# toposware/certificate-stark

Hardware: AMD Instinct MI355X
Metric: proofs/sec, state_transition AIR @ 2^20 steps (complete prove(): trace gen, LDE, Blake3 commitments, constraint evaluation, composition, DEEP, FRI, 96 queries) (higher is better)
Workload: dtype u64 (63-bit prime field, Montgomery) + u32 (Blake3)

## Files before the change

certificate-stark_amd/csrc/capi.hip:

```cpp
#include <hip/hip_runtime.h>
#include <stdio.h>
#include <stdlib.h>
#include <string.h>
#include <deque>
#include <new>
#include <vector>
#include "../../include/cstark.h"
#include "air_tx_host.h"
#include "blake3.h"
#include "ctx.h"
#include "constraints.h"
#include "deep.h"
#include "ext.h"
#include "generator_fold.h"
#include "hostfield.h"
#include "ntt.h"
#include "trace_gen.h"

namespace cs { thread_local char g_err[512] = ""; }
using cs::fail;
using cs::NttPlan;
using cs::CosetTable;
using cs::PeriodicTable;
using cs::g_err;
// ... 119 lines not shown
int lde_impl_inner(cstark_ctx *c, const uint64_t *d_coeffs, uint64_t *d_lde, uint32_t width, uint32_t col0, uint32_t ncols, uint32_t log_n,
                   uint32_t log_blowup, uint64_t domain_offset, uint32_t k0, uint32_t nk);
template <class F>
int lde_timed(cstark_ctx *c, uint64_t units, F &&run) {
    bool timed = c && c->part_timing && c->lde_ev_used + 2 <= LDE_EVENT_CAP;
    const size_t mark = timed ? c->lde_ev_used : 0;
    if (timed && lde_mark(c) != CSTARK_OK) { c->lde_ev_used = mark; timed = false; }
    const int rc = run();
    if (timed) {
        if (rc == CSTARK_OK && lde_mark(c) == CSTARK_OK) c->lde_units += units;
        else c->lde_ev_used = mark;
    }
    return rc;
}
int lde_impl(cstark_ctx *c, const uint64_t *d_coeffs, uint64_t *d_lde, uint32_t width, uint32_t col0, uint32_t ncols, uint32_t log_n, uint32_t log_blowup,
             uint64_t domain_offset, uint32_t k0, uint32_t nk) {
    return lde_timed(c, (uint64_t)ncols * nk << log_n, [&] { return lde_impl_inner(c, d_coeffs, d_lde, width, col0, ncols, log_n, log_blowup, domain_offset, k0, nk); });
}
int lde_impl_inner(cstark_ctx *c, const uint64_t *d_coeffs, uint64_t *d_lde, uint32_t width, uint32_t col0, uint32_t ncols, uint32_t log_n,
                   uint32_t log_blowup, uint64_t domain_offset, uint32_t k0, uint32_t nk) {
    if (!c || !d_coeffs || !d_lde || width == 0 || ncols == 0 || (uint64_t)col0 + ncols > width) return fail(CSTARK_ERR_INVALID_ARG, "cstark_lde_columns: bad argument");
    if (log_n < cs::NTT_MIN_LOG_N || log_n > cs::NTT_MAX_LOG_N || log_blowup > 6) return fail(CSTARK_ERR_UNSUPPORTED, "unsupported domain size");
    if (domain_offset == 0 || domain_offset >= cs::host::P) return fail(CSTARK_ERR_INVALID_ARG, "domain offset must be a nonzero field element");
    if ((uint64_t)k0 + nk > (1ull << log_blowup)) return fail(CSTARK_ERR_INVALID_ARG, "coset range exceeds the blowup factor");
    HIP_TRY(hipSetDevice(c->device));
    const NttPlan *p;
    const CosetTable *t;
    RC_TRY(get_plan(c, log_n, &p));
    RC_TRY(get_coset_table(c, log_n, log_blowup, domain_offset, &t));
    const size_t n = (size_t)1 << log_n;
    RC_TRY(ensure_ws(c, (size_t)width * n * 8));
    cs::NttArgs a{};
    a.in = d_coeffs + (size_t)col0 * n; a.scratch = (uint64_t *)c->ws;
    a.width = ncols; a.log_n = log_n;
    a.w = p->w; a.do_scale = false; a.aux = p->aux_w;
    if (nk > 1 && (size_t)nk * ncols * n * 8 <= LDE_BATCH_WS_BYTES) {
        if (ensure_ws(c, (size_t)nk * ncols * n * 8) == CSTARK_OK) {
            a.scratch = (uint64_t *)c->ws; a.out = d_lde + (size_t)col0 * n; a.batch = nk;
            a.prescale = t->s + (size_t)k0 * n; a.prescale_batch_stride = n;
            a.aux_ps = t->aux ? t->aux + (size_t)k0 * t->aux_words : nullptr; a.aux_ps_batch_stride = t->aux_words;
            a.in_batch_stride = 0; a.scratch_batch_stride = (size_t)ncols * n; a.out_batch_stride = (size_t)width * n;
            HIP_TRY(cs::ntt_columns(a, c->stream));
            return CSTARK_OK;
        }
        (void)hipGetLastError();
        RC_TRY(ensure_ws(c, (size_t)width * n * 8));
        a.scratch = (uint64_t *)c->ws;
    }
    a.batch = 1;
    for (uint32_t k = k0; k < k0 + nk; k++) {
        a.out = d_lde + ((size_t)(k - k0) * width + col0) * n;
        a.prescale = t->s + (size_t)k * n;
        a.aux_ps = t->aux ? t->aux + (size_t)k * t->aux_words : nullptr;
        HIP_TRY(cs::ntt_columns(a, c->stream));
    }
    return CSTARK_OK;
}

int get_step_table(cstark_ctx *c, unsigned log_n, unsigned log_b, uint64_t offset, unsigned log_block, unsigned split, const cs::StepTable **out) {
    for (const cs::StepTable &t : c->steps)
        if (t.log_n == log_n && t.log_b == log_b && t.offset == offset && t.log_block == log_block && t.split == split) { *out = &t; return CSTARK_OK; }
    const NttPlan *p;
    const CosetTable *ct;
    RC_TRY(get_plan(c, log_n, &p));
    RC_TRY(get_coset_table(c, log_n, log_b, offset, &ct));
    const size_t n = (size_t)1 << log_n, b = (size_t)1 << log_b;
    cs::StepTable t{log_n, log_b, offset, log_block, split, nullptr, nullptr};
    DevGuard g;
    HIP_TRY(g.alloc(&t.d, n * 8));
    HIP_TRY(g.alloc(&t.w, b * n * 8));
    cs::NttArgs a{};
    a.in = t.d; a.scratch = t.w; a.width = 1; a.batch = (unsigned)b; a.log_n = log_n;
    a.w = p->w; a.aux = p->aux_w;
    a.prescale = ct->s; a.prescale_batch_stride = n;
    a.aux_ps = ct->aux; a.aux_ps_batch_stride = ct->aux_words;
    a.in_batch_stride = 0; a.scratch_batch_stride = n;
    HIP_TRY(cs::ntt_step_build_tables(t.d, log_block, split, p->winv, a, c->stream));
    c->steps.push_back(t);
    g.release();
    *out = &c->steps.back();
    return CSTARK_OK;
}
int step_impl(cstark_ctx *c, uint64_t *d_evals, uint64_t *d_coeffs, uint64_t *d_lde, uint32_t width, uint32_t col0, uint32_t ncols, uint32_t log_n,
              uint32_t block_len, uint32_t split, uint32_t log_blowup, uint64_t domain_offset, uint32_t k0, uint32_t nk) {
    if (!c || !d_evals || !d_coeffs || !d_lde || width == 0 || ncols == 0 || (uint64_t)col0 + ncols > width)
        return fail(CSTARK_ERR_INVALID_ARG, "cstark_step_columns: bad argument");
    if (log_n < cs::NTT_MIN_LOG_N || log_n > cs::NTT_MAX_LOG_N || log_blowup > 6) return fail(CSTARK_ERR_UNSUPPORTED, "unsupported domain size");
    if (block_len == 0 || (block_len & (block_len - 1)) || block_len > (1u << log_n)) return fail(CSTARK_ERR_INVALID_ARG, "the block length must be a power of two up to the trace length");
    if (split >= block_len) return fail(CSTARK_ERR_INVALID_ARG, "the split row must lie inside the block");
    if (domain_offset == 0 || domain_offset >= cs::host::P) return fail(CSTARK_ERR_INVALID_ARG, "domain offset must be a nonzero field element");
    if ((uint64_t)k0 + nk > (1ull << log_blowup)) return fail(CSTARK_ERR_INVALID_ARG, "coset range exceeds the blowup factor");
    const size_t n = (size_t)1 << log_n;
    const unsigned log_block = (unsigned)__builtin_ctz(block_len);
    if (!cs::ntt_step_shape(log_n, log_block)) {
        RC_TRY(interpolate_impl(c, d_evals + (size_t)col0 * n, d_coeffs + (size_t)col0 * n, ncols, log_n));
        return lde_impl(c, d_coeffs, d_lde, width, col0, ncols, log_n, log_blowup, domain_offset, k0, nk);
    }
    HIP_TRY(hipSetDevice(c->device));
    const NttPlan *p;
    const cs::StepTable *t;
    RC_TRY(get_plan(c, log_n, &p));
    const cs::StepTable *tr = nullptr;
    RC_TRY(get_step_table(c, log_n, log_blowup, domain_offset, log_block, 0, &t));
    if (split) RC_TRY(get_step_table(c, log_n, log_blowup, domain_offset, log_block, split, &tr));
    RC_TRY(ensure_ws(c, ((size_t)ncols << (log_n - log_block)) * (split ? 16 : 8)));
    uint64_t *fac = (uint64_t *)c->ws;
    if (split)
        HIP_TRY(cs::ntt_step2_coefficients(d_evals + (size_t)col0 * n, fac, d_coeffs + (size_t)col0 * n, t->d, tr->d, ncols, log_n, log_block, split, p->winv,
                                           p->n_inv, c->stream));
    else
        HIP_TRY(cs::ntt_step_coefficients(d_evals + (size_t)col0 * n, fac, d_coeffs + (size_t)col0 * n, t->d, ncols, log_n, log_block, p->winv, p->n_inv, c->stream));
    return lde_timed(c, (uint64_t)ncols * nk << log_n, [&] {
        cs::NttArgs a{};
        a.out = d_lde + (size_t)col0 * n; a.width = ncols; a.batch = nk; a.log_n = log_n;
        a.out_batch_stride = (size_t)width * n; a.aux = p->aux_w;
        HIP_TRY(cs::ntt_step_rows(a, t->w + (size_t)k0 * n, tr ? tr->w + (size_t)k0 * n : nullptr, fac, log_block, c->stream));
        return (int)CSTARK_OK;
    });
}

int extend_periodic_columns(cstark_ctx *c, const std::vector<uint64_t> &cols, uint32_t ncols, uint32_t log_cycle, unsigned log_n, unsigned log_b,
                            DevGuard &keep, uint64_t **d_tab) {
    const size_t words = (size_t)ncols << log_cycle, n = (size_t)1 << log_n;
    uint64_t *d_cols = nullptr, *d_poly = nullptr;
    DevGuard tmp;
    HIP_TRY(tmp.alloc(&d_cols, words * 8));
    HIP_TRY(tmp.alloc(&d_poly, words * 8));
    HIP_TRY(keep.alloc(d_tab, (words << log_b) * 8));
    HIP_TRY(hipMemcpyAsync(d_cols, cols.data(), words * 8, hipMemcpyHostToDevice, c->stream));
    RC_TRY(interpolate_impl(c, d_cols, d_poly, ncols, log_cycle));
    RC_TRY(lde_impl(c, d_poly, *d_tab, ncols, 0, ncols, log_cycle, log_b, cs::host::pow(cs::host::lde_offset(), n >> log_cycle), 0, 1u << log_b));
    HIP_TRY(hipStreamSynchronize(c->stream));
    return CSTARK_OK;
}

int get_periodic(cstark_ctx *c, unsigned depth, unsigned log_n, unsigned log_b, const PeriodicTable **out) {
    for (const PeriodicTable &t : c->periodic)
        if (t.depth == depth && t.log_n == log_n && t.log_b == log_b) { *out = &t; return CSTARK_OK; }
    if (log_n < 10) return fail(CSTARK_ERR_INVALID_ARG, "the trace must hold at least one 1024-row transaction");
    std::vector<uint64_t> cols;
    if (!cs::host::tx_periodic_columns(depth, cols)) return fail(CSTARK_ERR_INVALID_ARG, "unsupported Merkle depth");
    static_assert(cs::host::TX_CYCLE == 1 << 10, "the cycle of TransactionAir's periodic columns");
    const size_t n = (size_t)1 << log_n, b = (size_t)1 << log_b;
    PeriodicTable t{depth, log_n, log_b, nullptr, nullptr, nullptr};
    DevGuard keep;
    RC_TRY(extend_periodic_columns(c, cols, cs::host::TX_NUM_PERIODIC, 10, log_n, log_b, keep, &t.tab));
    HIP_TRY(keep.alloc(&t.coset, b * cs::CE_COSET_CONSTS * 8));
    const uint64_t g = cs::host::lde_offset();
    std::vector<uint64_t> cc(b * cs::CE_COSET_CONSTS);
    const uint64_t wbn = cs::host::root_of_unity(log_n + log_b);
    uint64_t shift = g;
    for (size_t k = 0; k < b; k++) {
        uint64_t *o = cc.data() + k * cs::CE_COSET_CONSTS;
        o[0] = shift;
        o[1] = cs::host::inv(cs::host::sub(cs::host::pow(shift, n), cs::host::ONE));
        for (int gi = 0; gi < 5; gi++) o[2 + gi] = cs::host::pow(shift, cs::host::tx_group_adjustment(gi, n, n * b));
        o[7] = cs::host::pow(shift, cs::host::tx_boundary_adjustment(n, n * b));
        o[8] = cs::host::pow(shift, n - 1);
        o[9] = 0;
        shift = cs::host::mul(shift, wbn);
    }
    HIP_TRY(hipMemcpyAsync(t.coset, cc.data(), cc.size() * 8, hipMemcpyHostToDevice, c->stream));
    const NttPlan *plan;
    RC_TRY(get_plan(c, log_n, &plan));
    HIP_TRY(keep.alloc(&t.binv, b * 2 * n * 8));
    HIP_TRY(cs::build_boundary_inverses(t.binv, plan->w, t.coset, cs::host::inv(cs::host::root_of_unity(log_n)), log_n, log_b, c->stream));
    HIP_TRY(hipStreamSynchronize(c->stream));
    keep.release();
    c->periodic.push_back(t);
    *out = &c->periodic.back();
    return CSTARK_OK;
}

int get_small_periodic(cstark_ctx *c, int air, unsigned depth, unsigned log_n, unsigned log_b, const PeriodicTable **out) {
    for (const PeriodicTable &t : c->small_periodic)
        if (t.air == air && t.depth == depth && t.log_n == log_n && t.log_b == log_b) { *out = &t; return CSTARK_OK; }
    PeriodicTable t{depth, log_n, log_b, nullptr, nullptr, nullptr, air};
    std::vector<uint64_t> cols;
    DevGuard keep;
    if (air == CSTARK_AIR_MERKLE_UPDATE) {
        if (!cs::host::merkle_periodic_columns(depth, cols)) return fail(CSTARK_ERR_INVALID_ARG, "unsupported Merkle depth");
        RC_TRY(extend_periodic_columns(c, cols, 33, 9, log_n, log_b, keep, &t.tab));
    } else if (air == CSTARK_AIR_SCHNORR) {
        cs::host::schnorr_mask_columns(cols);
        RC_TRY(extend_periodic_columns(c, cols, 36, 9, log_n, log_b, keep, &t.tab));
    } else if (air == CSTARK_AIR_RESCUE_CHAIN) {
        using namespace cs::host;
        rescue_chain_periodic_columns(cols);
        const size_t n = (size_t)1 << log_n, b = (size_t)1 << log_b;
        for (int cidx = 0; cidx < 29; cidx++) intt_small(cols.data() + (size_t)cidx * 8, 3);
        std::vector<uint64_t> tab(b * 29 * 8);
        const uint64_t wbn = root_of_unity(log_n + log_b), w8 = root_of_unity(3);
        uint64_t shift = lde_offset();
        for (size_t k = 0; k < b; k++) {
// ... 225 lines not shown
    RC_TRY(tx_witness_reserve(c, n, d, sz, off));
    char *base = (char *)c->wit_buf;
    for (int i = 0; i < cs::WIT_NUM_SEGMENTS; i++)
        if (src[i]) HIP_TRY(hipMemcpyAsync(base + off[i], src[i], sz[i], hipMemcpyHostToDevice, c->stream));
    HIP_TRY(hipStreamSynchronize(c->stream));
    tx_witness_bind(c, n, d, off);
    return CSTARK_OK;
}

int cstark_tx_build_trace(cstark_ctx *c, uint64_t *d_trace) {
    if (!c || !d_trace) return fail(CSTARK_ERR_INVALID_ARG, "cstark_tx_build_trace: null argument");
    if (!c->wit_buf || c->wit.n_tx == 0) return fail(CSTARK_ERR_INVALID_ARG, "no witness uploaded");
    HIP_TRY(hipSetDevice(c->device));
    HIP_TRY(cs::launch_trace_gen(c->wit, d_trace, c->stream, c->side, c->ev_fork, c->ev_join));
    return CSTARK_OK;
}

uint64_t cstark_field_generator(void) { return cs::host::generator(); }
uint64_t cstark_field_lde_offset(void) { return cs::host::lde_offset(); }
uint64_t cstark_field_root_of_unity(uint32_t log_n) { return log_n <= 55 ? cs::host::root_of_unity(log_n) : 0; }

int cstark_interpolate_columns(cstark_ctx *c, uint64_t *d_evals, uint64_t *d_coeffs, uint32_t width, uint32_t log_n) {
    return interpolate_impl(c, d_evals, d_coeffs, width, log_n);
}
int cstark_lde_columns(cstark_ctx *c, const uint64_t *d_coeffs, uint64_t *d_lde, uint32_t width, uint32_t log_n, uint32_t log_blowup,
                       uint64_t domain_offset, uint32_t k0, uint32_t nk) {
    return lde_impl(c, d_coeffs, d_lde, width, 0, width, log_n, log_blowup, domain_offset, k0, nk);
}
int cstark_step_columns(cstark_ctx *c, uint64_t *d_evals, uint64_t *d_coeffs, uint64_t *d_lde, uint32_t width, uint32_t col0, uint32_t ncols,
                        uint32_t log_n, uint32_t block_len, uint32_t log_blowup, uint64_t domain_offset, uint32_t k0, uint32_t nk) {
    return step_impl(c, d_evals, d_coeffs, d_lde, width, col0, ncols, log_n, block_len, 0, log_blowup, domain_offset, k0, nk);
}
int cstark_step2_columns(cstark_ctx *c, uint64_t *d_evals, uint64_t *d_coeffs, uint64_t *d_lde, uint32_t width, uint32_t col0, uint32_t ncols,
                         uint32_t log_n, uint32_t block_len, uint32_t split, uint32_t log_blowup, uint64_t domain_offset, uint32_t k0, uint32_t nk) {
    if (split == 0) return fail(CSTARK_ERR_INVALID_ARG, "the split row must lie inside the block");
    return step_impl(c, d_evals, d_coeffs, d_lde, width, col0, ncols, log_n, block_len, split, log_blowup, domain_offset, k0, nk);
}

int cstark_composition_columns(cstark_ctx *c, const uint64_t *d_combined, uint64_t *d_cols, uint32_t log_n, uint32_t log_blowup) {
    if (!c || !d_combined || !d_cols) return fail(CSTARK_ERR_INVALID_ARG, "cstark_composition_columns: null argument");
    if (log_n < cs::NTT_MIN_LOG_N || log_n + log_blowup > cs::NTT_MAX_LOG_N || log_blowup == 0 || log_blowup > 6)
        return fail(CSTARK_ERR_UNSUPPORTED, "composition domain must be 2^7 .. 2^24 points");
    HIP_TRY(hipSetDevice(c->device));
    const size_t N = (size_t)1 << (log_n + log_blowup);
    RC_TRY(ensure_ws(c, 2 * N * 8));
    uint64_t *nat = (uint64_t *)c->ws, *h = nat + N;
    if (log_blowup <= 3) {
        const NttPlan *pn, *pN;
        RC_TRY(get_plan(c, log_n, &pn));
        RC_TRY(get_plan(c, log_n + log_blowup, &pN));
        cs::NttArgs a{};
        a.in = d_combined; a.scratch = h; a.out = nat; a.width = 1u << log_blowup; a.batch = 1; a.log_n = log_n;
        a.w = pn->winv; a.post_scale = pn->n_inv; a.do_scale = true; a.inverse = true; a.aux = pn->aux_winv;
        HIP_TRY(cs::ntt_columns(a, c->stream));
        const uint64_t b_inv = cs::host::inv(cs::host::from_u64(1ull << log_blowup));
        HIP_TRY(cs::coset_combine(nat, h, log_n, log_blowup, pN->winv, b_inv, c->stream));
        HIP_TRY(cs::split_columns(h, d_cols, log_n, log_blowup, cs::host::inv(cs::host::lde_offset()), c->stream));
        return CSTARK_OK;
    }
    HIP_TRY(cs::interleave_cosets(d_combined, nat, log_n, log_blowup, c->stream));
    const NttPlan *p;
    RC_TRY(get_plan(c, log_n + log_blowup, &p));
    cs::NttArgs a{};
    a.in = nat; a.scratch = nat; a.out = h; a.width = 1; a.batch = 1; a.log_n = log_n + log_blowup;
    a.w = p->winv; a.post_scale = p->n_inv; a.do_scale = true; a.inverse = true; a.aux = p->aux_winv;
    HIP_TRY(cs::ntt_columns(a, c->stream));
    HIP_TRY(cs::split_columns(h, d_cols, log_n, log_blowup, cs::host::inv(cs::host::lde_offset()), c->stream));
    return CSTARK_OK;
}

int cstark_evaluate_polys_at(cstark_ctx *c, const uint64_t *d_coeffs, uint32_t width, uint32_t log_n, const uint64_t *points, uint32_t npts,
                             uint64_t *out ) {
    if (!c || !d_coeffs || !points || !out || width == 0 || npts == 0 || npts > 16) return fail(CSTARK_ERR_INVALID_ARG, "cstark_evaluate_polys_at: bad argument");
    if (log_n > 30) return fail(CSTARK_ERR_INVALID_ARG, "bad polynomial size");
    HIP_TRY(hipSetDevice(c->device));
    const size_t need = ((size_t)npts + (size_t)npts * width + cs::poly_eval_scratch_words(width, log_n, npts)) * 8;
    if (need > c->desc_bytes) {
        if (c->desc_buf) { HIP_TRY(hipStreamSynchronize(c->stream)); HIP_TRY(hipFree(c->desc_buf)); c->desc_buf = nullptr; c->desc_bytes = 0; }
        HIP_TRY(hipMalloc(&c->desc_buf, need));
        c->desc_bytes = need;
    }
    uint64_t *d_pts = (uint64_t *)c->desc_buf, *d_out = d_pts + npts, *d_scr = d_out + (size_t)npts * width;
    HIP_TRY(hipMemcpyAsync(d_pts, points, (size_t)npts * 8, hipMemcpyHostToDevice, c->stream));
    HIP_TRY(cs::poly_eval(d_coeffs, width, log_n, d_pts, npts, d_out, d_scr, c->stream));
    HIP_TRY(hipMemcpyAsync(out, d_out, (size_t)npts * width * 8, hipMemcpyDeviceToHost, c->stream));
    HIP_TRY(cs::stream_wait(c->stream));
    return CSTARK_OK;
}

int cstark_deep_composition(cstark_ctx *c, const uint64_t *d_trace_lde, const uint64_t *d_comp_lde, uint32_t width, uint32_t n_comp,
                            uint64_t z, const uint64_t *ood_trace, const uint64_t *ood_comp, const uint64_t *alpha, const uint64_t *beta,
                            const uint64_t *delta, uint64_t deg_a, uint64_t deg_b, uint64_t *d_out, uint32_t log_n, uint32_t log_blowup,
                            uint32_t k0, uint32_t nk) {
    if (!c || !d_trace_lde || !d_comp_lde || !ood_trace || !ood_comp || !alpha || !beta || !delta || !d_out || nk == 0 || width == 0 || n_comp == 0)
        return fail(CSTARK_ERR_INVALID_ARG, "cstark_deep_composition: bad argument");
    if (log_n < cs::NTT_MIN_LOG_N || log_n > cs::NTT_MAX_LOG_N || log_blowup > 6 || (uint64_t)k0 + nk > (1ull << log_blowup)) return fail(CSTARK_ERR_INVALID_ARG, "bad domain parameters");
    HIP_TRY(hipSetDevice(c->device));
    const NttPlan *plan;
    RC_TRY(get_plan(c, log_n, &plan));
    const size_t b = (size_t)1 << log_blowup, nco = 2 * (size_t)width + n_comp, words = 2 * nco + b;
    if (c->deep_words < words) {
        HIP_TRY(hipStreamSynchronize(c->stream));
        if (c->deep_buf) { HIP_TRY(hipFree(c->deep_buf)); c->deep_buf = nullptr; }
        if (c->deep_stage) { HIP_TRY(hipHostFree(c->deep_stage)); c->deep_stage = nullptr; }
        c->deep_words = 0;
        HIP_TRY(hipMalloc((void **)&c->deep_buf, words * 8));
        HIP_TRY(hipHostMalloc((void **)&c->deep_stage, words * 8, hipHostMallocDefault));
        if (!c->deep_ev) HIP_TRY(hipEventCreateWithFlags(&c->deep_ev, hipEventDisableTiming));
        c->deep_words = words;
    } else {
        HIP_TRY(hipEventSynchronize(c->deep_ev));
    }
    uint64_t *blk = c->deep_stage;
    memcpy(blk, alpha, width * 8); memcpy(blk + width, beta, width * 8); memcpy(blk + 2 * width, delta, n_comp * 8);
    memcpy(blk + nco, ood_trace, 2 * (size_t)width * 8); memcpy(blk + nco + 2 * width, ood_comp, n_comp * 8);
    const uint64_t wbn = cs::host::root_of_unity(log_n + log_blowup);
    uint64_t shift = cs::host::lde_offset();
    for (size_t k = 0; k < b; k++) { blk[2 * nco + k] = shift; shift = cs::host::mul(shift, wbn); }
    HIP_TRY(hipMemcpyAsync(c->deep_buf, blk, words * 8, hipMemcpyHostToDevice, c->stream));
    HIP_TRY(hipEventRecord(c->deep_ev, c->stream));
    const uint64_t *d = c->deep_buf;
    cs::DeepParams p{};
    p.trace_lde = d_trace_lde; p.comp_lde = d_comp_lde; p.w = plan->w; p.coef = d; p.ood = d + nco; p.shifts = d + 2 * nco; p.out = d_out;
    p.z = z; p.zw = cs::host::mul(z, cs::host::root_of_unity(log_n)); p.zb = cs::host::pow(z, n_comp);
    p.deg_a = deg_a; p.deg_b = deg_b; p.width = width; p.nb = n_comp; p.log_n = log_n; p.k0 = k0;
    HIP_TRY(cs::deep_composition(p, nk, c->stream));
    return CSTARK_OK;
}

int cstark_interleave_cosets(cstark_ctx *c, const uint64_t *d_coset_major, uint64_t *d_natural, uint32_t log_n, uint32_t log_blowup) {
    if (!c || !d_coset_major || !d_natural || d_coset_major == d_natural) return fail(CSTARK_ERR_INVALID_ARG, "cstark_interleave_cosets: bad argument");
    if (log_n + log_blowup > 30 || log_blowup > 6) return fail(CSTARK_ERR_INVALID_ARG, "bad domain parameters");
    HIP_TRY(hipSetDevice(c->device));
    HIP_TRY(cs::interleave_cosets(d_coset_major, d_natural, log_n, log_blowup, c->stream));
    return CSTARK_OK;
}
int cstark_fri_fold4(cstark_ctx *c, const uint64_t *d_evals, uint64_t *d_out, uint32_t log_n, uint64_t domain_offset, uint64_t alpha) {
    if (!c || !d_evals || !d_out || d_evals == d_out) return fail(CSTARK_ERR_INVALID_ARG, "cstark_fri_fold4: bad argument");
    if (log_n < cs::NTT_MIN_LOG_N || log_n > cs::NTT_MAX_LOG_N) return fail(CSTARK_ERR_UNSUPPORTED, "layer size must be 2^6 .. 2^24");
    if (domain_offset == 0 || domain_offset >= cs::host::P || alpha >= cs::host::P) return fail(CSTARK_ERR_INVALID_ARG, "offset / alpha must be field elements");
    HIP_TRY(hipSetDevice(c->device));
    const NttPlan *p;
    RC_TRY(get_plan(c, log_n, &p));
    HIP_TRY(cs::fri_fold4(d_evals, d_out, log_n, p->winv, cs::host::inv(domain_offset), alpha, cs::host::inv(cs::host::from_u64(4)), c->stream));
    return CSTARK_OK;
}
int cstark_fri_fold(cstark_ctx *c, const uint64_t *d_evals, uint64_t *d_out, uint32_t log_n, uint32_t folding_factor, uint64_t domain_offset, uint64_t alpha) {
    if (!c || !d_evals || !d_out || d_evals == d_out) return fail(CSTARK_ERR_INVALID_ARG, "cstark_fri_fold: bad argument");
    if (folding_factor != 4 && folding_factor != 8 && folding_factor != 16) return fail(CSTARK_ERR_UNSUPPORTED, "FRI folding factor must be 4, 8 or 16");
    if (log_n < cs::NTT_MIN_LOG_N || log_n > cs::NTT_MAX_LOG_N) return fail(CSTARK_ERR_UNSUPPORTED, "layer size must be 2^6 .. 2^24");
    if (domain_offset == 0 || domain_offset >= cs::host::P || alpha >= cs::host::P) return fail(CSTARK_ERR_INVALID_ARG, "offset / alpha must be field elements");
    HIP_TRY(hipSetDevice(c->device));
    const NttPlan *p;
    RC_TRY(get_plan(c, log_n, &p));
    const unsigned log_f = folding_factor == 4 ? 2 : folding_factor == 8 ? 3 : 4;
    HIP_TRY(cs::fri_fold(d_evals, d_out, log_n, log_f, p->winv, cs::host::inv(domain_offset), alpha, cs::host::inv(cs::host::from_u64(folding_factor)), c->stream));
    return CSTARK_OK;
}

int cstark_evaluate_polys_at_ext(cstark_ctx *c, const uint64_t *d_coeffs, uint32_t width, uint32_t log_n, uint32_t m, const uint64_t *z, uint64_t *out) {
    if (!c || !d_coeffs || !z || !out || width == 0 || (m != 2 && m != 3)) return fail(CSTARK_ERR_INVALID_ARG, "cstark_evaluate_polys_at_ext: bad argument");
    if (log_n > 30) return fail(CSTARK_ERR_INVALID_ARG, "bad polynomial size");
    for (uint32_t i = 0; i < m; i++) if (z[i] >= cs::host::P) return fail(CSTARK_ERR_INVALID_ARG, "the point is not an extension element");
    HIP_TRY(hipSetDevice(c->device));
    const size_t need = ((size_t)m * width + cs::poly_eval_ext_scratch_words(width, log_n, m)) * 8;
    if (need > c->desc_bytes) {
        if (c->desc_buf) { HIP_TRY(hipStreamSynchronize(c->stream)); HIP_TRY(hipFree(c->desc_buf)); c->desc_buf = nullptr; c->desc_bytes = 0; }
        HIP_TRY(hipMalloc(&c->desc_buf, need));
        c->desc_bytes = need;
    }
    uint64_t *d_out = (uint64_t *)c->desc_buf, *d_scr = d_out + (size_t)m * width;
    HIP_TRY(cs::poly_eval_ext(d_coeffs, width, log_n, z, m, d_out, d_scr, c->stream));
    HIP_TRY(hipMemcpyAsync(out, d_out, (size_t)m * width * 8, hipMemcpyDeviceToHost, c->stream));
    HIP_TRY(cs::stream_wait(c->stream));
    return CSTARK_OK;
}
}

int fri_coin_fold_dev(cstark_ctx *c, uint32_t *d_seed, const uint8_t *d_root, uint64_t *d_alpha, uint32_t *d_root_out, const uint64_t *d_evals,
                      uint64_t *d_out, uint32_t log_n, uint32_t log_f, uint64_t domain_offset, uint32_t m) {
    if (log_n < cs::NTT_MIN_LOG_N || log_n > cs::NTT_MAX_LOG_N) return fail(CSTARK_ERR_UNSUPPORTED, "layer size must be 2^6 .. 2^24");
    if (m < 1 || m > 3) return fail(CSTARK_ERR_INVALID_ARG, "fri_coin_fold_dev: bad extension degree");
    const NttPlan *p;
    RC_TRY(get_plan(c, log_n, &p));
    const uint64_t offset_inv = cs::host::inv(domain_offset), inv_f = cs::host::inv(cs::host::from_u64(1ull << log_f));
    if (m == 1) {
        HIP_TRY(cs::fri_coin(d_seed, d_root, d_alpha, d_root_out, c->stream));
        HIP_TRY(cs::fri_fold(d_evals, d_out, log_n, log_f, p->winv, offset_inv, 0, inv_f, c->stream, d_alpha));
    } else {
        HIP_TRY(cs::fri_coin_ext(d_seed, d_root, d_alpha, d_root_out, m, c->stream));
        HIP_TRY(cs::fri_fold_ext(d_evals, d_out, log_n, log_f, p->winv, offset_inv, nullptr, m, inv_f, c->stream, d_alpha));
    }
    return CSTARK_OK;
}
int hash_rows_slots(cstark_ctx *c, uint32_t hash_fn, const uint64_t *d_lde, uint8_t *d_leaves, uint32_t width, uint32_t log_n, uint32_t log_blowup, uint32_t log_s) {
    if (!c || !d_lde || !d_leaves || width == 0 || width > 128 || hash_fn > 1 || log_blowup > 6 || log_s > log_blowup || ((uintptr_t)d_leaves & 15) != 0)
        return fail(CSTARK_ERR_INVALID_ARG, "hash_rows_slots: bad argument");
    HIP_TRY(hipSetDevice(c->device));
    if (hash_fn == 1) HIP_TRY(cs::hash_rows_sha3(d_lde, d_leaves, width, log_n, log_blowup, 0, 1u << log_blowup, c->stream, log_s));
    else HIP_TRY(cs::hash_rows(d_lde, d_leaves, width, log_n, log_blowup, 0, 1u << log_blowup, c->stream, log_s));
    return CSTARK_OK;
}
int evaluate_ood_frames(cstark_ctx *c, const uint64_t *d_coeffs, uint32_t width, const uint64_t *d_ccoef, uint32_t n_comp, uint32_t log_n,
                        const uint64_t zpts[2], uint64_t zb, uint64_t *out_trace, uint64_t *out_comp) {
    if (!c || !d_coeffs || !d_ccoef || !out_trace || !out_comp || width == 0 || n_comp == 0) return fail(CSTARK_ERR_INVALID_ARG, "evaluate_ood_frames: bad argument");
    HIP_TRY(hipSetDevice(c->device));
    const size_t n_out = 2 * (size_t)width + n_comp;
    const size_t scr_t = cs::poly_eval_scratch_words(width, log_n, 2), scr_c = cs::poly_eval_scratch_words(n_comp, log_n, 1);
    const size_t need = (4 + n_out + scr_t + scr_c) * 8;
    if (need > c->desc_bytes) {
        if (c->desc_buf) { HIP_TRY(hipStreamSynchronize(c->stream)); HIP_TRY(hipFree(c->desc_buf)); c->desc_buf = nullptr; c->desc_bytes = 0; }
        HIP_TRY(hipMalloc(&c->desc_buf, need));
        c->desc_bytes = need;
    }
    uint64_t *d_pts = (uint64_t *)c->desc_buf, *d_out = d_pts + 4, *d_scr = d_out + n_out;
    const uint64_t pts[3] = {zpts[0], zpts[1], zb};
    HIP_TRY(hipMemcpyAsync(d_pts, pts, sizeof pts, hipMemcpyHostToDevice, c->stream));
    HIP_TRY(cs::poly_eval(d_coeffs, width, log_n, d_pts, 2, d_out, d_scr, c->stream));
    HIP_TRY(cs::poly_eval(d_ccoef, n_comp, log_n, d_pts + 2, 1, d_out + 2 * (size_t)width, d_scr + scr_t, c->stream));
    std::vector<uint64_t> host(n_out);
    HIP_TRY(hipMemcpyAsync(host.data(), d_out, n_out * 8, hipMemcpyDeviceToHost, c->stream));
    HIP_TRY(cs::stream_wait(c->stream));
    memcpy(out_trace, host.data(), 2 * (size_t)width * 8);
    memcpy(out_comp, host.data() + 2 * (size_t)width, (size_t)n_comp * 8);
    return CSTARK_OK;
}

int ood_frames_dev(cstark_ctx *c, const uint64_t *d_coeffs, uint32_t width, const uint64_t *d_ccoef, uint32_t n_comp, uint32_t log_n, const uint64_t *d_pts,
                   uint64_t *d_out) {
    if (!c || !d_coeffs || !d_ccoef || !d_pts || !d_out || width == 0 || n_comp == 0) return fail(CSTARK_ERR_INVALID_ARG, "ood_frames_dev: bad argument");
    HIP_TRY(hipSetDevice(c->device));
    const size_t scr_t = cs::poly_eval_scratch_words(width, log_n, 2), scr_c = cs::poly_eval_scratch_words(n_comp, log_n, 1);
    const size_t need = (scr_t + scr_c) * 8;
    if (need > c->desc_bytes) {
        if (c->desc_buf) { HIP_TRY(hipStreamSynchronize(c->stream)); HIP_TRY(hipFree(c->desc_buf)); c->desc_buf = nullptr; c->desc_bytes = 0; }
        HIP_TRY(hipMalloc(&c->desc_buf, need));
        c->desc_bytes = need;
    }
    uint64_t *d_scr = (uint64_t *)c->desc_buf;
    HIP_TRY(cs::poly_eval(d_coeffs, width, log_n, d_pts, 2, d_out, d_scr, c->stream));
    HIP_TRY(cs::poly_eval(d_ccoef, n_comp, log_n, d_pts + 2, 1, d_out + 2 * (size_t)width, d_scr + scr_t, c->stream));
    return CSTARK_OK;
}
int desc_reserve(cstark_ctx *c, size_t bytes) {
    if (bytes <= c->desc_bytes) return CSTARK_OK;
    if (c->desc_buf) { HIP_TRY(hipStreamSynchronize(c->stream)); HIP_TRY(hipFree(c->desc_buf)); c->desc_buf = nullptr; c->desc_bytes = 0; }
    HIP_TRY(hipMalloc(&c->desc_buf, bytes));
    c->desc_bytes = bytes;
    return CSTARK_OK;
}
static size_t ood_scratch_words(uint32_t width, uint32_t n_comp, uint32_t log_n, uint32_t m, size_t *scr_t, size_t *scr_c) {
    if (m == 1) { *scr_t = cs::poly_eval_scratch_words(width, log_n, 2); *scr_c = cs::poly_eval_scratch_words(n_comp, log_n, 1); return *scr_t + *scr_c; }
    *scr_t = cs::poly_eval_ext_scratch_words(width, log_n, m); *scr_c = cs::poly_eval_ext_scratch_words(m * n_comp, log_n, m);
    return 2 * *scr_t + *scr_c + (size_t)m * m * n_comp;
}
size_t ood_frames_dev_scratch_bytes(uint32_t width, uint32_t n_comp, uint32_t log_n, uint32_t m) {
    size_t scr_t, scr_c;
    return ood_scratch_words(width, n_comp, log_n, m, &scr_t, &scr_c) * 8;
}
int ood_frames_dev_ext(cstark_ctx *c, const uint64_t *d_coeffs, uint32_t width, const uint64_t *d_ccoef, uint32_t n_comp, uint32_t log_n, uint32_t m,
                       const uint64_t *d_pts, uint64_t *d_out) {
    if (!c || !d_coeffs || !d_ccoef || !d_pts || !d_out || width == 0 || n_comp == 0 || (m != 2 && m != 3)) return fail(CSTARK_ERR_INVALID_ARG, "ood_frames_dev_ext: bad argument");
    HIP_TRY(hipSetDevice(c->device));
    size_t scr_t, scr_c;
    RC_TRY(desc_reserve(c, ood_scratch_words(width, n_comp, log_n, m, &scr_t, &scr_c) * 8));
    uint64_t *d_scr = (uint64_t *)c->desc_buf, *d_raw = d_scr + 2 * scr_t + scr_c;
    const size_t mw = (size_t)m * width;
    HIP_TRY(cs::poly_eval_ext(d_coeffs, width, log_n, nullptr, m, d_out, d_scr, c->stream, d_pts));
    HIP_TRY(cs::poly_eval_ext(d_coeffs, width, log_n, nullptr, m, d_out + mw, d_scr + scr_t, c->stream, d_pts + m));
    HIP_TRY(cs::poly_eval_ext(d_ccoef, m * n_comp, log_n, nullptr, m, d_raw, d_scr + 2 * scr_t, c->stream, d_pts + 2 * m));
    HIP_TRY(cs::ood_recombine_ext(d_raw, d_out + 2 * mw, n_comp, m, c->stream));
    return CSTARK_OK;
}
int deep_composition_ext_dev(cstark_ctx *c, const uint64_t *d_trace_lde, const uint64_t *d_comp_lde, uint32_t width, uint32_t n_comp, uint32_t m,
                             const uint64_t *d_coef, const uint64_t *d_ood, uint64_t *d_scal, const uint64_t *d_shifts, uint64_t *d_out, uint32_t log_n,
                             uint32_t log_blowup, uint32_t nk) {
    if (!c || !d_trace_lde || !d_comp_lde || !d_coef || !d_ood || !d_scal || !d_shifts || !d_out || width == 0 || n_comp == 0 || (m != 2 && m != 3))
        return fail(CSTARK_ERR_INVALID_ARG, "deep_composition_ext_dev: bad argument");
    if (log_n < cs::NTT_MIN_LOG_N || log_n > cs::NTT_MAX_LOG_N || log_blowup > 6 || nk == 0 || nk > (1u << log_blowup)) return fail(CSTARK_ERR_INVALID_ARG, "bad domain parameters");
    HIP_TRY(hipSetDevice(c->device));
    const NttPlan *plan;
    RC_TRY(get_plan(c, log_n, &plan));
    HIP_TRY(cs::deep_ext_consts(d_coef, d_ood, d_scal, width, n_comp, m, c->stream));
    cs::DeepExtParams p{};
    p.trace_lde = d_trace_lde; p.comp_lde = d_comp_lde; p.w = plan->w; p.coef = d_coef; p.shifts = d_shifts; p.out = d_out; p.scal = d_scal;
    p.width = width; p.nb = n_comp; p.log_n = log_n; p.log_b = log_blowup; p.m = m;
    p.nk = nk == (1u << log_blowup) ? 0 : nk;
    HIP_TRY(cs::deep_composition_ext(p, c->stream));
    return CSTARK_OK;
}
int deep_composition_ext_cosets(cstark_ctx *c, const uint64_t *d_trace_lde, const uint64_t *d_comp_lde, uint32_t width, uint32_t n_comp, uint32_t m,
                                const uint64_t *z, const uint64_t *ood_trace, const uint64_t *ood_comp, const uint64_t *alpha, const uint64_t *beta,
                                const uint64_t *delta, const uint64_t *deg_a, const uint64_t *deg_b, uint64_t *d_out, uint32_t log_n, uint32_t log_blowup,
                                uint32_t nk) {
    if (!c || !d_trace_lde || !d_comp_lde || !z || !ood_trace || !ood_comp || !alpha || !beta || !delta || !deg_a || !deg_b || !d_out || width == 0 || n_comp == 0 ||
        (m != 2 && m != 3))
        return fail(CSTARK_ERR_INVALID_ARG, "cstark_deep_composition_ext: bad argument");
    if (log_n < cs::NTT_MIN_LOG_N || log_n > cs::NTT_MAX_LOG_N || log_blowup > 6) return fail(CSTARK_ERR_INVALID_ARG, "bad domain parameters");
    using namespace cs::host;
    HIP_TRY(hipSetDevice(c->device));
    const NttPlan *plan;
    RC_TRY(get_plan(c, log_n, &plan));
    const size_t b = (size_t)1 << log_blowup, nco = (size_t)m * (2 * (size_t)width + n_comp);
    std::vector<uint64_t> blk(nco + b);
    memcpy(blk.data(), alpha, (size_t)m * width * 8);
    memcpy(blk.data() + (size_t)m * width, beta, (size_t)m * width * 8);
    memcpy(blk.data() + (size_t)2 * m * width, delta, (size_t)m * n_comp * 8);
    const uint64_t wbn = root_of_unity(log_n + log_blowup);
    uint64_t shift = lde_offset();
    for (size_t k = 0; k < b; k++) { blk[nco + k] = shift; shift = mul(shift, wbn); }
    const size_t bytes = blk.size() * 8;
    if (bytes > c->desc_bytes) {
        if (c->desc_buf) { HIP_TRY(hipStreamSynchronize(c->stream)); HIP_TRY(hipFree(c->desc_buf)); c->desc_buf = nullptr; c->desc_bytes = 0; }
        HIP_TRY(hipMalloc(&c->desc_buf, bytes));
        c->desc_bytes = bytes;
    }
    HIP_TRY(hipMemcpyAsync(c->desc_buf, blk.data(), bytes, hipMemcpyHostToDevice, c->stream));
    HIP_TRY(cs::stream_wait(c->stream));
    cs::DeepExtParams p{};
    p.trace_lde = d_trace_lde; p.comp_lde = d_comp_lde; p.w = plan->w; p.coef = (const uint64_t *)c->desc_buf; p.shifts = p.coef + nco; p.out = d_out;
    const EX zz = ex_load(z, m), zw = ex_scale(zz, root_of_unity(log_n)), zb = ex_pow(zz, n_comp, m), da = ex_load(deg_a, m), db = ex_load(deg_b, m);
    EX k1 = ex_zero(), k2 = ex_zero(), k3 = ex_zero();
    for (uint32_t i = 0; i < width; i++) {
        k1 = ex_add(k1, ex_mul(ex_load(alpha + (size_t)m * i, m), ex_load(ood_trace + (size_t)m * i, m), m));
// ... 21 lines not shown
int cstark_fri_fold4_ext(cstark_ctx *c, const uint64_t *d_evals, uint64_t *d_out, uint32_t log_n, uint64_t domain_offset, uint32_t m, const uint64_t *alpha) {
    if (!c || !d_evals || !d_out || !alpha || d_evals == d_out || (m != 2 && m != 3)) return fail(CSTARK_ERR_INVALID_ARG, "cstark_fri_fold4_ext: bad argument");
    if (log_n < cs::NTT_MIN_LOG_N || log_n > cs::NTT_MAX_LOG_N) return fail(CSTARK_ERR_UNSUPPORTED, "layer size must be 2^6 .. 2^24");
    if (domain_offset == 0 || domain_offset >= cs::host::P) return fail(CSTARK_ERR_INVALID_ARG, "offset must be a nonzero field element");
    for (uint32_t i = 0; i < m; i++) if (alpha[i] >= cs::host::P) return fail(CSTARK_ERR_INVALID_ARG, "alpha is not an extension element");
    HIP_TRY(hipSetDevice(c->device));
    const NttPlan *p;
    RC_TRY(get_plan(c, log_n, &p));
    HIP_TRY(cs::fri_fold4_ext(d_evals, d_out, log_n, p->winv, cs::host::inv(domain_offset), alpha, m, cs::host::inv(cs::host::from_u64(4)), c->stream));
    return CSTARK_OK;
}
int cstark_fri_fold_ext(cstark_ctx *c, const uint64_t *d_evals, uint64_t *d_out, uint32_t log_n, uint32_t folding_factor, uint64_t domain_offset, uint32_t m,
                        const uint64_t *alpha) {
    if (!c || !d_evals || !d_out || !alpha || d_evals == d_out || (m != 2 && m != 3)) return fail(CSTARK_ERR_INVALID_ARG, "cstark_fri_fold_ext: bad argument");
    if (folding_factor != 4 && folding_factor != 8 && folding_factor != 16) return fail(CSTARK_ERR_UNSUPPORTED, "FRI folding factor must be 4, 8 or 16");
    if (log_n < cs::NTT_MIN_LOG_N || log_n > cs::NTT_MAX_LOG_N) return fail(CSTARK_ERR_UNSUPPORTED, "layer size must be 2^6 .. 2^24");
    if (domain_offset == 0 || domain_offset >= cs::host::P) return fail(CSTARK_ERR_INVALID_ARG, "offset must be a nonzero field element");
    for (uint32_t i = 0; i < m; i++) if (alpha[i] >= cs::host::P) return fail(CSTARK_ERR_INVALID_ARG, "alpha is not an extension element");
    HIP_TRY(hipSetDevice(c->device));
    const NttPlan *p;
    RC_TRY(get_plan(c, log_n, &p));
    const unsigned log_f = folding_factor == 4 ? 2 : folding_factor == 8 ? 3 : 4;
    HIP_TRY(cs::fri_fold_ext(d_evals, d_out, log_n, log_f, p->winv, cs::host::inv(domain_offset), alpha, m, cs::host::inv(cs::host::from_u64(folding_factor)), c->stream));
    return CSTARK_OK;
}

int cstark_hash_rows(cstark_ctx *c, const uint64_t *d_lde, uint8_t *d_leaves, uint32_t width, uint32_t log_n, uint32_t log_blowup,
                     uint32_t k0, uint32_t nk) {
    if (!c || !d_lde || !d_leaves) return fail(CSTARK_ERR_INVALID_ARG, "cstark_hash_rows: null argument");
    if (width == 0 || width > 128) return fail(CSTARK_ERR_UNSUPPORTED, "row width must be 1..128 elements (single Blake3 chunk)");
    if (log_n > 30 || log_blowup > 6 || (uint64_t)k0 + nk > (1ull << log_blowup)) return fail(CSTARK_ERR_INVALID_ARG, "bad domain parameters");
    if (((uintptr_t)d_leaves & 15) != 0) return fail(CSTARK_ERR_INVALID_ARG, "d_leaves must be 16-byte aligned");
    HIP_TRY(hipSetDevice(c->device));
    HIP_TRY(cs::hash_rows(d_lde, d_leaves, width, log_n, log_blowup, k0, nk, c->stream));
    return CSTARK_OK;
}

int cstark_hash_rows_fn(cstark_ctx *c, uint32_t hash_fn, const uint64_t *d_lde, uint8_t *d_leaves, uint32_t width, uint32_t log_n, uint32_t log_blowup,
                        uint32_t k0, uint32_t nk) {
    if (hash_fn == 0) return cstark_hash_rows(c, d_lde, d_leaves, width, log_n, log_blowup, k0, nk);
    if (hash_fn != 1) return fail(CSTARK_ERR_UNSUPPORTED, "hash_fn must be 0 (Blake3_256) or 1 (Sha3_256)");
    if (!c || !d_lde || !d_leaves) return fail(CSTARK_ERR_INVALID_ARG, "cstark_hash_rows_fn: null argument");
    if (width == 0 || width > 128) return fail(CSTARK_ERR_UNSUPPORTED, "row width must be 1..128 elements");
    if (log_n > 30 || log_blowup > 6 || (uint64_t)k0 + nk > (1ull << log_blowup)) return fail(CSTARK_ERR_INVALID_ARG, "bad domain parameters");
    if (((uintptr_t)d_leaves & 15) != 0) return fail(CSTARK_ERR_INVALID_ARG, "d_leaves must be 16-byte aligned");
    HIP_TRY(hipSetDevice(c->device));
    HIP_TRY(cs::hash_rows_sha3(d_lde, d_leaves, width, log_n, log_blowup, k0, nk, c->stream));
    return CSTARK_OK;
}
int cstark_merkle_build_fn(cstark_ctx *c, uint32_t hash_fn, uint8_t *d_nodes, uint32_t log_leaves) {
    if (hash_fn == 0) return cstark_merkle_build(c, d_nodes, log_leaves);
    if (hash_fn != 1) return fail(CSTARK_ERR_UNSUPPORTED, "hash_fn must be 0 (Blake3_256) or 1 (Sha3_256)");
    if (!c || !d_nodes) return fail(CSTARK_ERR_INVALID_ARG, "cstark_merkle_build_fn: null argument");
    if (log_leaves == 0 || log_leaves > 30) return fail(CSTARK_ERR_INVALID_ARG, "tree must have 2 .. 2^30 leaves");
    if (((uintptr_t)d_nodes & 15) != 0) return fail(CSTARK_ERR_INVALID_ARG, "d_nodes must be 16-byte aligned");
    HIP_TRY(hipSetDevice(c->device));
    HIP_TRY(cs::merkle_build_sha3(d_nodes, log_leaves, c->stream));
    return CSTARK_OK;
}

int cstark_merkle_build(cstark_ctx *c, uint8_t *d_nodes, uint32_t log_leaves) {
    if (!c || !d_nodes) return fail(CSTARK_ERR_INVALID_ARG, "cstark_merkle_build: null argument");
    if (log_leaves == 0 || log_leaves > 30) return fail(CSTARK_ERR_INVALID_ARG, "tree must have 2 .. 2^30 leaves");
    if (((uintptr_t)d_nodes & 15) != 0) return fail(CSTARK_ERR_INVALID_ARG, "d_nodes must be 16-byte aligned");
    HIP_TRY(hipSetDevice(c->device));
    HIP_TRY(cs::merkle_build(d_nodes, log_leaves, c->stream));
    return CSTARK_OK;
}

int cstark_tx_evaluate_transitions(cstark_ctx *c, const uint64_t *d_lde, uint64_t *d_out, uint32_t merkle_depth, uint32_t log_n,
                                   uint32_t log_blowup, uint32_t k0, uint32_t nk) {
    cs::CeParams p;
    RC_TRY(ce_params(c, d_lde, d_out, merkle_depth, log_n, log_blowup, k0, nk, &p));
    HIP_TRY(cs::launch_eval_transitions(p, nk, c->stream));
    return CSTARK_OK;
}

}
int lde_column_range(cstark_ctx *c, const uint64_t *d_coeffs, uint64_t *d_lde, uint32_t width, uint32_t col0, uint32_t ncols, uint32_t log_n,
                     uint32_t log_blowup, uint64_t domain_offset, uint32_t k0, uint32_t nk) {
    return lde_impl(c, d_coeffs, d_lde, width, col0, ncols, log_n, log_blowup, domain_offset, k0, nk);
}
int step_column_range(cstark_ctx *c, uint64_t *d_evals, uint64_t *d_coeffs, uint64_t *d_lde, uint32_t width, uint32_t col0, uint32_t ncols, uint32_t log_n,
                      uint32_t block_len, uint32_t split, uint32_t log_blowup, uint64_t domain_offset, uint32_t k0, uint32_t nk) {
    return step_impl(c, d_evals, d_coeffs, d_lde, width, col0, ncols, log_n, block_len, split, log_blowup, domain_offset, k0, nk);
}
int tx_build_trace_split(cstark_ctx *c, uint64_t *d_trace) {
    if (!c || !d_trace) return fail(CSTARK_ERR_INVALID_ARG, "tx_build_trace_split: null argument");
    if (!c->wit_buf || c->wit.n_tx == 0) return fail(CSTARK_ERR_INVALID_ARG, "no witness uploaded");
    HIP_TRY(hipSetDevice(c->device));
    HIP_TRY(cs::launch_trace_gen_split(c->wit, d_trace, c->stream, c->side, c->side2, c->ev_fork, c->ev_join, c->ev_mid, c->ev_join2));
    return CSTARK_OK;
}
static constexpr size_t TX_COEF_WORDS = (size_t)cs::CE_MAX_SETS * cs::CE_COEF_WORDS;
static int ensure_coef_buf(cstark_ctx *c) {
    static_assert(sizeof(cstark_tx_coeffs) == cs::CE_COEF_WORDS * 8, "coefficient block layout");
    if (!c->coef_buf) HIP_TRY(hipMalloc((void **)&c->coef_buf, (TX_COEF_WORDS + (size_t)cs::CE_MAX_SETS * cs::CE_RTAB_WORDS) * 8));
    return CSTARK_OK;
}
int tx_coef_device_block(cstark_ctx *c, uint64_t **d_coef) {
    HIP_TRY(hipSetDevice(c->device));
    RC_TRY(ensure_coef_buf(c));
    *d_coef = c->coef_buf;
    return CSTARK_OK;
}
static int upload_coeffs(cstark_ctx *c, const cstark_tx_coeffs *coeffs, uint32_t m, cs::CeParams &p) {
    constexpr size_t COEF_WORDS = TX_COEF_WORDS;
    RC_TRY(ensure_coef_buf(c));
    if (!c->coef_stage) {
        if (!c->coef_ev) HIP_TRY(hipEventCreateWithFlags(&c->coef_ev, hipEventDisableTiming));
        HIP_TRY(hipHostMalloc(&c->coef_stage, (size_t)cs::CE_MAX_SETS * sizeof(cstark_tx_coeffs), hipHostMallocDefault));
    } else {
        HIP_TRY(hipEventSynchronize(c->coef_ev));
    }
    memcpy(c->coef_stage, coeffs, (size_t)m * sizeof(cstark_tx_coeffs));
    HIP_TRY(hipMemcpyAsync(c->coef_buf, c->coef_stage, (size_t)m * sizeof(cstark_tx_coeffs), hipMemcpyHostToDevice, c->stream));
    HIP_TRY(hipEventRecord(c->coef_ev, c->stream));
    p.coef = c->coef_buf;
    p.rtab = c->coef_buf + COEF_WORDS;
    p.m = m;
    return CSTARK_OK;
}

struct SplitMerge { unsigned log_n = 0; cs::CosetMergeDesc desc; cs::CosetMergeTerm hi; };
static const SplitMerge &tx_split_merge(unsigned log_n) {
    static thread_local SplitMerge sm;
    if (sm.log_n == log_n) return sm;
    const uint64_t n = 1ull << log_n, g = cs::host::lde_offset();
    uint64_t adj[3];
    for (int i = 0; i < 3; i++) adj[i] = cs::host::tx_group_adjustment(i, n, 8 * n);
    static const int first[cs::CE_SPLIT_FAMILIES] = {0, cs::CE_SPLIT_FAM0, 7, 9, 11}, count[cs::CE_SPLIT_FAMILIES] = {4, 3, 2, 2, 2};
    sm.desc = cs::CosetMergeDesc{};
    sm.desc.families = cs::CE_SPLIT_FAMILIES;
    sm.desc.tables_per_set = cs::CE_SPLIT_TABLES;
    sm.desc.raw_family = cs::CE_SPLIT_FAMILIES - 1;
    for (int f = 0; f < cs::CE_SPLIT_FAMILIES; f++) {
        sm.desc.terms[f] = count[f];
        for (int t = 0; t < count[f]; t++) sm.desc.term[f][t] = cs::coset_merge_term(first[f] + t, t ? adj[t - 1] : 0, log_n, g);
    }
    sm.hi = cs::coset_merge_term(0, adj[0], log_n, cs::host::mul(g, cs::host::root_of_unity(log_n + 3)), 2);
    sm.log_n = log_n;
    return sm;
}

namespace {

struct SplitStage {
    unsigned log_n;
    size_t n;
    const NttPlan *pn, *p4, *p8;
    const CosetTable *t1;
    hipStream_t stream;
};
int split_stage(cstark_ctx *c, unsigned log_n, SplitStage *s) {
    *s = SplitStage{log_n, (size_t)1 << log_n, nullptr, nullptr, nullptr, nullptr, c->stream};
    RC_TRY(get_plan(c, log_n, &s->pn));
    RC_TRY(get_plan(c, log_n + 2, &s->p4));
    RC_TRY(get_plan(c, log_n + 3, &s->p8));
    return get_coset_table(c, log_n, 3, cs::host::from_u64(1), &s->t1);
}

int inverse_columns(const SplitStage &s, const uint64_t *in, uint64_t *scratch, uint64_t *out, unsigned width, unsigned batch = 1, size_t batch_stride = 0) {
    cs::NttArgs a{};
    a.in = in; a.scratch = scratch; a.out = out; a.width = width; a.batch = batch; a.log_n = s.log_n;
    a.in_batch_stride = batch_stride; a.scratch_batch_stride = batch_stride; a.out_batch_stride = batch_stride;
    a.w = s.pn->winv; a.post_scale = s.pn->n_inv; a.do_scale = true; a.inverse = true; a.aux = s.pn->aux_winv;
    HIP_TRY(cs::ntt_columns(a, s.stream));
    return CSTARK_OK;
// ... 710 lines not shown
```

certificate-stark_amd/csrc/ctx.h:

```cpp
#pragma once
#include <stdlib.h>
#include <hip/hip_runtime.h>
#include <stdio.h>
#include <deque>
#include <vector>
#include "../../include/cstark.h"
#include "constraints.h"
#include "trace_gen.h"
#include "witness_layout.h"

#include <chrono>
namespace cs {
inline hipError_t stream_wait(hipStream_t st) {
    static const bool block = [] { const char *e = getenv("CSTARK_SYNC_BLOCK"); return e && atoi(e) != 0; }();
    static const long spin_us = [] { const char *e = getenv("CSTARK_SPIN_US"); return e ? atol(e) : 200L; }();
    if (block || spin_us <= 0) return hipStreamSynchronize(st);
    const auto t0 = std::chrono::steady_clock::now();
    hipError_t e;
    for (unsigned it = 0; (e = hipStreamQuery(st)) == hipErrorNotReady; it++) {
#if defined(__x86_64__) || defined(__i386__)
        __builtin_ia32_pause();
#endif
        if ((it & 15) == 15 && std::chrono::duration_cast<std::chrono::microseconds>(std::chrono::steady_clock::now() - t0).count() > spin_us)
            return hipStreamSynchronize(st);
    }
    return e;
}
inline hipError_t stream_wait_tail(hipStream_t st, hipEvent_t near_end) {
    static const bool block = [] { const char *e = getenv("CSTARK_SYNC_BLOCK"); return e && atoi(e) != 0; }();
    if (block) return hipStreamSynchronize(st);
    hipError_t e = hipEventSynchronize(near_end);
    if (e != hipSuccess) return e;
    const auto t0 = std::chrono::steady_clock::now();
    for (unsigned it = 0; (e = hipStreamQuery(st)) == hipErrorNotReady; it++) {
#if defined(__x86_64__) || defined(__i386__)
        __builtin_ia32_pause();
#endif
        if ((it & 15) == 15 && std::chrono::duration_cast<std::chrono::microseconds>(std::chrono::steady_clock::now() - t0).count() > 5000)
            return hipStreamSynchronize(st);
    }
    return e;
}
}

namespace cs {

extern thread_local char g_err[512];

inline int fail(int code, const char *fmt, const char *detail = "") {
    snprintf(g_err, sizeof g_err, fmt, detail);
    return code;
}
#define HIP_TRY(expr)                                                                                                              \
    do {                                                                                                                           \
        hipError_t e_ = (expr);                                                                                                    \
        if (e_ != hipSuccess) return cs::fail(e_ == hipErrorOutOfMemory ? CSTARK_ERR_OOM : CSTARK_ERR_HIP, #expr ": %s", hipGetErrorString(e_)); \
    } while (0)
#define RC_TRY(expr)            \
    do {                        \
        int rc_ = (expr);       \
        if (rc_) return rc_;    \
    } while (0)

int grind_search(hipStream_t stream, unsigned long long *d_found, const uint8_t seed[32], uint32_t hash_fn, unsigned bits, uint64_t chunk, uint64_t *nonce_out);

struct NttPlan {
    unsigned log_n;
    uint64_t *w, *winv;
    uint64_t n_inv;
    uint64_t *aux_w = nullptr, *aux_winv = nullptr;
};
struct CosetTable {
    unsigned log_n, log_b;
    uint64_t offset;
    uint64_t *s;
    uint64_t *aux = nullptr;
    size_t aux_words = 0;
};
struct StepTable {
    unsigned log_n, log_b;
    uint64_t offset;
    unsigned log_block;
    unsigned split;
    uint64_t *d;
    uint64_t *w;
};
struct PeriodicTable {
    unsigned depth, log_n, log_b;
    uint64_t *tab;
    uint64_t *coset;
    uint64_t *binv;
    int air = 0;
};
struct AssertInverseTable {
    unsigned log_n, log_b;
// ... 39 lines not shown
    int device = 0;
    hipStream_t stream = nullptr;
    bool owns_stream = false;
    hipStream_t side = nullptr, side2 = nullptr;
    hipEvent_t ev_fork = nullptr, ev_join = nullptr, ev_join2 = nullptr, ev_mid = nullptr;
    void *wit_buf = nullptr;
    size_t wit_bytes = 0;
    cs::TxWitnessDev wit{};
    std::deque<cs::NttPlan> plans;
    std::deque<cs::CosetTable> cosets;
    std::deque<cs::StepTable> steps;
    std::deque<cs::PeriodicTable> periodic;
    uint64_t *coef_buf = nullptr;
    uint64_t *gfold_j = nullptr;
    void *coef_stage = nullptr;
    hipEvent_t coef_ev = nullptr;
    std::deque<cs::AssertInverseTable> assert_inv;
    std::deque<cs::AirCombineStatic> air_static;
    uint64_t *air_coef_buf = nullptr, *air_coef_stage = nullptr;
    size_t air_coef_words = 0;
    hipEvent_t air_coef_ev = nullptr;
    uint64_t *deep_buf = nullptr, *deep_stage = nullptr;
    size_t deep_words = 0;
    hipEvent_t deep_ev = nullptr;
    std::deque<cs::PeriodicTable> small_periodic;
    void *desc_buf = nullptr;
    hipEvent_t part_ev[cs::CE_NUM_PARTS + 1] = {};
    bool part_timing = false, part_valid = false;
    std::vector<hipEvent_t> lde_ev;
    size_t lde_ev_used = 0;
    uint64_t lde_units = 0;
    uint64_t *tail_buf = nullptr;
    std::vector<uint64_t> schnorr_rx;
    std::vector<uint64_t> schnorr_av_stage;
    std::vector<uint64_t> schnorr_pub;
    std::vector<uint8_t> schnorr_s;
    uint8_t schnorr_seed[32] = {}, schnorr_seed_key[12] = {};
    size_t tail_bytes = 0;
    size_t desc_bytes = 0;
    cs::ProveArena *arena = nullptr;
    cs::VerifyArena *verify = nullptr;
    void *ws = nullptr;
    size_t ws_bytes = 0;
    uint64_t *shard_bit37 = nullptr;
    size_t shard_bit37_words = 0;
    void *rb_dev = nullptr, *rb_host = nullptr;
    size_t rb_dev_bytes = 0, rb_host_bytes = 0;
    void *sig_buf = nullptr;
    size_t sig_bytes = 0;
};
int signature_check(cstark_ctx *c, const char *who, uint32_t count, const uint64_t *messages, const uint64_t *sig_rx, const uint8_t *sig_s,
                    uint8_t *verdicts, uint64_t *rx_out);
int tx_witness_reserve(cstark_ctx *c, size_t n, size_t d, size_t *sz, size_t *off);
void tx_witness_bind(cstark_ctx *c, size_t n, size_t d, const size_t *off);
int fri_coin_fold_dev(cstark_ctx *c, uint32_t *d_seed, const uint8_t *d_root, uint64_t *d_alpha, uint32_t *d_root_out, const uint64_t *d_evals,
                      uint64_t *d_out, uint32_t log_n, uint32_t log_f, uint64_t domain_offset, uint32_t m);
int hash_rows_slots(cstark_ctx *c, uint32_t hash_fn, const uint64_t *d_lde, uint8_t *d_leaves, uint32_t width, uint32_t log_n, uint32_t log_blowup, uint32_t log_s);
struct cstark_gather_desc {
    const void *src;
    void *out;
    const uint32_t *d_pos, *d_count;
    uint32_t paths, a, log_n, log_b, log_s, count, lvl0;
};
int gather_jobs_launch(cstark_ctx *c, const cstark_gather_desc *jobs, uint32_t n_jobs);
int plan_tables(cstark_ctx *c, unsigned log_n, const uint64_t **w, const uint64_t **winv);

struct cstark_tx_coeffs;
int tx_evaluate_constraints_sets(cstark_ctx *c, const uint64_t *d_lde, const cstark_tx_coeffs *coeffs, uint32_t m, const uint64_t pub_inputs[4],
                                 uint64_t *const *d_outs, uint32_t merkle_depth, uint32_t log_n, uint32_t log_blowup, uint32_t k0, uint32_t nk,
                                 bool input_is_lde, const uint64_t *d_pub = nullptr);
int tx_coef_device_block(cstark_ctx *c, uint64_t **d_coef);
int air_stage(cstark_ctx *c, const cs::AirStageRequest &rq);
int tx_evaluate_constraints_shard(cstark_ctx *c, const uint64_t *d_lde, const uint64_t *d_coeffs, const cstark_tx_coeffs *coeffs, const uint64_t pub_inputs[4],
                                  uint64_t *d_out, uint32_t merkle_depth, uint32_t log_n, uint32_t k0, uint32_t nk);
int tx_shard_combine(cstark_ctx *c, const uint64_t *d_parts, uint64_t *d_out, uint32_t log_n, uint32_t nk);
constexpr uint32_t TX_LATE_COLS = 37;
constexpr uint32_t TX_ROOT_COLS = 58;
constexpr uint32_t TX_COPY_COLS = 65;
constexpr uint32_t TX_STEP_COLS = 27;
int tx_build_trace_split(cstark_ctx *c, uint64_t *d_trace);
int lde_column_range(cstark_ctx *c, const uint64_t *d_coeffs, uint64_t *d_lde, uint32_t width, uint32_t col0, uint32_t ncols, uint32_t log_n,
                     uint32_t log_blowup, uint64_t domain_offset, uint32_t k0, uint32_t nk);
int step_column_range(cstark_ctx *c, uint64_t *d_evals, uint64_t *d_coeffs, uint64_t *d_lde, uint32_t width, uint32_t col0, uint32_t ncols, uint32_t log_n,
                      uint32_t block_len, uint32_t split, uint32_t log_blowup, uint64_t domain_offset, uint32_t k0, uint32_t nk);
int evaluate_ood_frames(cstark_ctx *c, const uint64_t *d_coeffs, uint32_t width, const uint64_t *d_ccoef, uint32_t n_comp, uint32_t log_n,
                        const uint64_t zpts[2], uint64_t zb, uint64_t *out_trace, uint64_t *out_comp);
int ood_frames_dev(cstark_ctx *c, const uint64_t *d_coeffs, uint32_t width, const uint64_t *d_ccoef, uint32_t n_comp, uint32_t log_n, const uint64_t *d_pts,
                   uint64_t *d_out);
int desc_reserve(cstark_ctx *c, size_t bytes);
size_t ood_frames_dev_scratch_bytes(uint32_t width, uint32_t n_comp, uint32_t log_n, uint32_t m);
int ood_frames_dev_ext(cstark_ctx *c, const uint64_t *d_coeffs, uint32_t width, const uint64_t *d_ccoef, uint32_t n_comp, uint32_t log_n, uint32_t m,
                       const uint64_t *d_pts, uint64_t *d_out);
int deep_composition_ext_dev(cstark_ctx *c, const uint64_t *d_trace_lde, const uint64_t *d_comp_lde, uint32_t width, uint32_t n_comp, uint32_t m,
                             const uint64_t *d_coef, const uint64_t *d_ood, uint64_t *d_scal, const uint64_t *d_shifts, uint64_t *d_out, uint32_t log_n,
                             uint32_t log_blowup, uint32_t nk);
int deep_composition_ext_cosets(cstark_ctx *c, const uint64_t *d_trace_lde, const uint64_t *d_comp_lde, uint32_t width, uint32_t n_comp, uint32_t m,
                                const uint64_t *z, const uint64_t *ood_trace, const uint64_t *ood_comp, const uint64_t *alpha, const uint64_t *beta,
                                const uint64_t *delta, const uint64_t *deg_a, const uint64_t *deg_b, uint64_t *d_out, uint32_t log_n, uint32_t log_blowup,
                                uint32_t nk);
```

certificate-stark_amd/csrc/deep.h:

```cpp
#pragma once
#include <hip/hip_runtime.h>
#include <stddef.h>
#include <stdint.h>

namespace cs {

struct DeepParams {
    const uint64_t *trace_lde, *comp_lde;
    const uint64_t *w, *shifts;
    const uint64_t *coef;
    const uint64_t *ood;
    uint64_t *out;
    uint64_t z, zw, zb, deg_a, deg_b;
    uint32_t width, nb, log_n, k0;
    const uint64_t *scal;
};

size_t poly_eval_scratch_words(unsigned width, unsigned log_n, unsigned npts);
hipError_t poly_eval(const uint64_t *d_coeffs, unsigned width, unsigned log_n, const uint64_t *d_points, unsigned npts, uint64_t *d_out,
                     uint64_t *d_scratch, hipStream_t stream);
hipError_t deep_composition(const DeepParams &p, unsigned nk, hipStream_t stream);
hipError_t fri_fold4(const uint64_t *d_evals, uint64_t *d_out, unsigned log_n, const uint64_t *d_winv, uint64_t offset_inv, uint64_t alpha,
                     uint64_t inv4, hipStream_t stream, const uint64_t *d_alpha = nullptr);
hipError_t fri_fold(const uint64_t *d_evals, uint64_t *d_out, unsigned log_n, unsigned log_f, const uint64_t *d_winv, uint64_t offset_inv, uint64_t alpha,
                    uint64_t inv_f, hipStream_t stream, const uint64_t *d_alpha = nullptr);

}
```

certificate-stark_amd/csrc/deep.hip:

```cpp
#include "deep.h"
#include "fp.cuh"

namespace cs {
namespace {

#ifndef CS_PE_SEG
#define CS_PE_SEG 16384
#endif
constexpr int PE_SEG = CS_PE_SEG, PE_MAXPTS = 2;
template <int NP>
__global__ __launch_bounds__(256) void k_poly_eval_partial(const fp *__restrict__ coeffs, size_t n, const fp *__restrict__ points, fp *__restrict__ partial,
                                                           unsigned width, unsigned seg_len) {
    __shared__ fp part[NP][256];
    const unsigned segs = gridDim.x, seg = blockIdx.x, col = blockIdx.y, t = threadIdx.x;
    const fp *c = coeffs + (size_t)col * n + (size_t)seg * seg_len;
    fp z[NP], z256[NP], acc[NP];
#pragma unroll
    for (int p = 0; p < NP; p++) { z[p] = points[p]; z256[p] = fp_pow(z[p], 256); acc[p] = 0; }
    const unsigned per = (seg_len + 255) / 256;
    for (unsigned k = per; k-- > 0;) {
        const fp v = k * 256 + t < seg_len ? c[(size_t)k * 256 + t] : 0;
#pragma unroll
        for (int p = 0; p < NP; p++) acc[p] = fp_add(fp_mul(acc[p], z256[p]), v);
    }
#pragma unroll
    for (int p = 0; p < NP; p++) part[p][t] = fp_mul(acc[p], fp_pow(z[p], (uint64_t)seg * seg_len + t));
    __syncthreads();
    for (int s = 128; s > 0; s >>= 1) {
        if ((int)t < s) {
#pragma unroll
            for (int p = 0; p < NP; p++) part[p][t] = fp_add(part[p][t], part[p][t + s]);
        }
        __syncthreads();
    }
    if (t < NP) partial[((size_t)t * width + col) * segs + seg] = part[t][0];
}
__global__ void k_poly_eval_sum(const fp *__restrict__ partial, fp *__restrict__ out, unsigned total, unsigned segs) {
    const unsigned i = blockIdx.x * blockDim.x + threadIdx.x;
    if (i >= total) return;
    fp a = 0;
    for (unsigned s = 0; s < segs; s++) a = fp_add(a, partial[(size_t)i * segs + s]);
    out[i] = a;
}

__global__ __launch_bounds__(256) void k_deep(DeepParams p) {
    const size_t n = (size_t)1 << p.log_n;
    const size_t j = blockIdx.x * (size_t)256 + threadIdx.x;
    if (j >= n) return;
    const unsigned kk = blockIdx.y;
    const fp x = fp_mul(p.shifts[p.k0 + kk], p.w[j]);
    const fp pz = p.scal ? p.scal[0] : p.z, pzw = p.scal ? p.scal[1] : p.zw, pzb = p.scal ? p.scal[2] : p.zb;
    const fp d1 = fp_sub(x, pz), d2 = fp_sub(x, pzw), d3 = fp_sub(x, pzb);
    const fp inv = fp_inv(fp_mul(fp_mul(d1, d2), d3));
    const fp i1 = fp_mul(inv, fp_mul(d2, d3)), i2 = fp_mul(inv, fp_mul(d1, d3)), i3 = fp_mul(inv, fp_mul(d1, d2));
    Acc128 s1 = acc_zero(), s2 = acc_zero(), s3 = acc_zero();
    const fp *t = p.trace_lde + (size_t)kk * p.width * n + j;
    for (unsigned c = 0; c < p.width; c++) {
        const fp v = t[(size_t)c * n];
        acc_mad(s1, p.coef[c], fp_sub(v, p.ood[c]));
        acc_mad(s2, p.coef[p.width + c], fp_sub(v, p.ood[p.width + c]));
        if ((c & 3) == 3) { acc_fold(s1); acc_fold(s2); }
    }
    acc_fold(s1); acc_fold(s2);
    const fp *h = p.comp_lde + (size_t)kk * p.nb * n + j;
    for (unsigned i = 0; i < p.nb; i++) {
        acc_mad(s3, p.coef[2 * p.width + i], fp_sub(h[(size_t)i * n], p.ood[2 * p.width + i]));
        if ((i & 3) == 3) acc_fold(s3);
    }
    acc_fold(s3);
    fp acc = fp_add(fp_add(fp_mul(acc_reduce(s1), i1), fp_mul(acc_reduce(s2), i2)), fp_mul(acc_reduce(s3), i3));
    const fp dga = p.scal ? p.scal[3] : p.deg_a, dgb = p.scal ? p.scal[4] : p.deg_b;
    p.out[(size_t)kk * n + j] = fp_mul(acc, fp_add(dga, fp_mul(dgb, x)));
}

__global__ __launch_bounds__(256) void k_fri_fold4(const fp *__restrict__ evals, fp *__restrict__ out, size_t q, const fp *__restrict__ winv,
                                                   fp offset_inv, fp alpha, fp inv4, const fp *__restrict__ alpha_dev) {
    const size_t i = blockIdx.x * (size_t)256 + threadIdx.x;
    if (i >= q) return;
    if (alpha_dev) alpha = *alpha_dev;
    const fp v0 = evals[i], v1 = evals[i + q], v2 = evals[i + 2 * q], v3 = evals[i + 3 * q];
    const fp zi = winv[q];
    const fp a = fp_add(v0, v2), b = fp_sub(v0, v2), c = fp_add(v1, v3), d = fp_mul(fp_sub(v1, v3), zi);
    const fp s0 = fp_add(a, c), s2 = fp_sub(a, c), s1 = fp_add(b, d), s3 = fp_sub(b, d);
    const fp r = fp_mul(alpha, fp_mul(offset_inv, winv[i]));
    const fp r2 = fp_sqr(r), r3 = fp_mul(r2, r);
    fp acc = fp_add(fp_add(s0, fp_mul(r, s1)), fp_add(fp_mul(r2, s2), fp_mul(r3, s3)));
    out[i] = fp_mul(acc, inv4);
}

template <int LOG_F>
__global__ __launch_bounds__(256) void k_fri_fold(const fp *__restrict__ evals, fp *__restrict__ out, size_t q, const fp *__restrict__ winv,
                                                  fp offset_inv, fp alpha, fp inv_f, const fp *__restrict__ alpha_dev) {
    constexpr int F = 1 << LOG_F;
    const size_t i = blockIdx.x * (size_t)256 + threadIdx.x;
    if (i >= q) return;
    if (alpha_dev) alpha = *alpha_dev;
    fp v[F];
#pragma unroll
    for (int t = 0; t < F; t++) v[t] = evals[i + (size_t)t * q];
#pragma unroll
    for (int len = F; len >= 2; len >>= 1) {
        const int half = len >> 1, step = F / len;
#pragma unroll
        for (int base = 0; base < F; base += len) {
#pragma unroll
            for (int t = 0; t < half; t++) {
                const fp a = v[base + t], b = v[base + t + half];
                v[base + t] = fp_add(a, b);
                const fp d = fp_sub(a, b);
                v[base + t + half] = (t == 0) ? d : fp_mul(d, winv[(size_t)(t * step) * q]);
            }
        }
    }
    const fp r = fp_mul(alpha, fp_mul(offset_inv, winv[i]));
    fp acc = 0;
#pragma unroll
    for (int k = F - 1; k >= 0; k--) {
        int br = 0;
#pragma unroll
        for (int bit = 0; bit < LOG_F; bit++) br |= ((k >> bit) & 1) << (LOG_F - 1 - bit);
        acc = fp_add(fp_mul(acc, r), v[br]);
    }
    out[i] = fp_mul(acc, inv_f);
}

}

hipError_t fri_fold4(const uint64_t *d_evals, uint64_t *d_out, unsigned log_n, const uint64_t *d_winv, uint64_t offset_inv, uint64_t alpha,
                     uint64_t inv4, hipStream_t stream, const uint64_t *d_alpha) {
    const size_t q = ((size_t)1 << log_n) / 4;
    hipLaunchKernelGGL(k_fri_fold4, dim3((unsigned)((q + 255) / 256)), dim3(256), 0, stream, d_evals, d_out, q, d_winv, offset_inv, alpha, inv4, d_alpha);
    return hipGetLastError();
}
hipError_t fri_fold(const uint64_t *d_evals, uint64_t *d_out, unsigned log_n, unsigned log_f, const uint64_t *d_winv, uint64_t offset_inv, uint64_t alpha,
                    uint64_t inv_f, hipStream_t stream, const uint64_t *d_alpha) {
    if (log_f == 2) return fri_fold4(d_evals, d_out, log_n, d_winv, offset_inv, alpha, inv_f, stream, d_alpha);
    if ((log_f != 3 && log_f != 4) || log_n < log_f) return hipErrorInvalidValue;
    const size_t q = ((size_t)1 << log_n) >> log_f;
    const dim3 grid((unsigned)((q + 255) / 256));
    if (log_f == 3) hipLaunchKernelGGL(k_fri_fold<3>, grid, dim3(256), 0, stream, d_evals, d_out, q, d_winv, offset_inv, alpha, inv_f, d_alpha);
    else hipLaunchKernelGGL(k_fri_fold<4>, grid, dim3(256), 0, stream, d_evals, d_out, q, d_winv, offset_inv, alpha, inv_f, d_alpha);
    return hipGetLastError();
}

size_t poly_eval_scratch_words(unsigned width, unsigned log_n, unsigned npts) {
    const size_t n = (size_t)1 << log_n, seg = n < (size_t)PE_SEG ? n : (size_t)PE_SEG;
    return (size_t)npts * width * (n / seg);
}
hipError_t poly_eval(const uint64_t *d_coeffs, unsigned width, unsigned log_n, const uint64_t *d_points, unsigned npts, uint64_t *d_out,
                     uint64_t *d_scratch, hipStream_t stream) {
    const size_t n = (size_t)1 << log_n;
    const unsigned seg_len = (unsigned)(n < (size_t)PE_SEG ? n : (size_t)PE_SEG), segs = (unsigned)(n / seg_len);
    for (unsigned p0 = 0; p0 < npts; p0 += PE_MAXPTS) {
        const unsigned np = npts - p0 >= 2 ? 2 : 1;
        fp *part = d_scratch + (size_t)p0 * width * segs;
        if (np == 2) hipLaunchKernelGGL(k_poly_eval_partial<2>, dim3(segs, width), dim3(256), 0, stream, d_coeffs, n, d_points + p0, part, width, seg_len);
        else hipLaunchKernelGGL(k_poly_eval_partial<1>, dim3(segs, width), dim3(256), 0, stream, d_coeffs, n, d_points + p0, part, width, seg_len);
    }
    const unsigned total = npts * width;
    hipLaunchKernelGGL(k_poly_eval_sum, dim3((total + 255) / 256), dim3(256), 0, stream, d_scratch, d_out, total, segs);
    return hipGetLastError();
}
hipError_t deep_composition(const DeepParams &p, unsigned nk, hipStream_t stream) {
    const size_t n = (size_t)1 << p.log_n;
    hipLaunchKernelGGL(k_deep, dim3((unsigned)((n + 255) / 256), nk), dim3(256), 0, stream, p);
    return hipGetLastError();
}

}
```

certificate-stark_amd/csrc/ntt.hip:

```cpp
#include "ntt.h"
#include "fp.cuh"
#include "hostfield.h"
#include "../../include/cstark_conventions.h"
#ifdef CS_NTT_NOMATH
#define fp_mul(a, b) ((a) ^ (b))
#define fp_add(a, b) ((a) + (b))
#define fp_sub(a, b) ((a) - (b))
#define fp_sub_lazy(a, b) ((a) - (b))
#endif
#ifndef CS_NTT_SKIP
#define CS_NTT_SKIP 0
#endif

namespace cs {
namespace {

__device__ __forceinline__ fp mb_load(const fp *row, unsigned lane_off, unsigned fake) { return (CS_NTT_SKIP & 16) ? (fp)fake : row[lane_off]; }
__device__ __forceinline__ void mb_store(fp *row, unsigned lane_off, fp val) {
    if (!(CS_NTT_SKIP & 8) || val == 0x123456789abcdefull) row[lane_off] = val;
}
constexpr bool MB_NO_TWIDDLE_FILL = (CS_NTT_SKIP & 1) != 0, MB_NO_PRESCALE = (CS_NTT_SKIP & 2) != 0, MB_NO_OUTPUT_FACTOR = (CS_NTT_SKIP & 4) != 0;

constexpr int NT = 256;

// ... 1110 lines not shown
    return hipGetLastError();
}

bool ntt_step_shape(unsigned log_n, unsigned log_block) {
    NttThreeStepShape s;
    return log_block < log_n && ntt_three_step_shape(log_n, &s) && log_n - log_block <= s.log_c;
}
namespace {
__global__ __launch_bounds__(256) void k_step_d(fp *__restrict__ d, const fp *__restrict__ winv, size_t n, unsigned log_t) {
    const size_t k = blockIdx.x * (size_t)256 + threadIdx.x;
    if (k >= n) return;
    d[k] = k == 0 ? FP_ONE : (k & (((size_t)1 << log_t) - 1)) == 0 ? 0 : fp_inv(fp_sub(winv[k], FP_ONE));
}
__global__ __launch_bounds__(256) void k_step_dr(fp *__restrict__ d, const fp *__restrict__ winv, size_t n, unsigned split, fp r_mont) {
    const size_t k = blockIdx.x * (size_t)256 + threadIdx.x;
    if (k >= n) return;
    d[k] = k == 0 ? r_mont : fp_mul(fp_sub(winv[(k * split) & (n - 1)], FP_ONE), fp_inv(fp_sub(winv[k], FP_ONE)));
}
__global__ __launch_bounds__(NT) void k_step_factors(const fp *__restrict__ evals, fp *__restrict__ fac, unsigned log_n, unsigned log_t,
                                                     const fp *__restrict__ winv, fp n_inv, fp t_inv) {
    extern __shared__ __attribute__((aligned(16))) fp smem[];
    const unsigned T = 1u << log_t, log_block = log_n - log_t;
    fp *tile = smem, *tw = smem + T;
    const fp *col = evals + ((size_t)blockIdx.x << log_n);
    for (unsigned t = threadIdx.x; t < T; t += NT) tile[t] = col[(size_t)t << log_block];
    for (unsigned e = threadIdx.x; e < T / 2; e += NT) tw[e] = winv[(size_t)e << log_block];
    __syncthreads();
    lds_ntt_dif<1>(tile, log_t, tw);
    for (unsigned j = threadIdx.x; j < T; j += NT) {
        const fp g = tile[bitrev(j, log_t)];
        fac[((size_t)blockIdx.x << log_t) + j] = j == 0 ? fp_mul(g, t_inv) : fp_mul(fp_mul(g, n_inv), fp_sub(winv[(size_t)j << log_block], FP_ONE));
    }
}
__global__ __launch_bounds__(NT) void k_step2_factors(const fp *__restrict__ evals, fp *__restrict__ fac, unsigned log_n, unsigned log_t, unsigned split,
                                                      const fp *__restrict__ winv, fp n_inv, fp t_inv) {
    extern __shared__ __attribute__((aligned(16))) fp smem[];
    const unsigned T = 1u << log_t, log_block = log_n - log_t;
    fp *tile = smem, *tile_d = smem + T, *tw = smem + 2 * T;
    const fp *col = evals + ((size_t)blockIdx.x << log_n);
    for (unsigned t = threadIdx.x; t < T; t += NT) {
        const fp v = col[((size_t)t << log_block) + split];
        tile[t] = v;
        tile_d[t] = fp_sub(col[(size_t)t << log_block], v);
    }
    for (unsigned e = threadIdx.x; e < T / 2; e += NT) tw[e] = winv[(size_t)e << log_block];
    __syncthreads();
    lds_ntt_dif<1>(tile, log_t, tw);
    lds_ntt_dif<1>(tile_d, log_t, tw);
    fp *out = fac + ((size_t)blockIdx.x << (log_t + 1));
    for (unsigned j = threadIdx.x; j < T; j += NT) {
        const fp g = tile[bitrev(j, log_t)];
        out[j] = j == 0 ? fp_mul(g, t_inv) : fp_mul(fp_mul(g, n_inv), fp_sub(winv[(size_t)j << log_block], FP_ONE));
        out[T + j] = fp_mul(tile_d[bitrev(j, log_t)], n_inv);
    }
}
__global__ __launch_bounds__(256) void k_step2_coeffs(const fp *__restrict__ fac, const fp *__restrict__ d, const fp *__restrict__ dr, fp *__restrict__ coeffs,
                                                      unsigned log_n, unsigned log_t) {
    const size_t k = blockIdx.x * (size_t)256 + threadIdx.x, j = k & (((size_t)1 << log_t) - 1);
    const fp *f = fac + ((size_t)blockIdx.y << (log_t + 1));
    coeffs[((size_t)blockIdx.y << log_n) + k] = fp_add(fp_mul(f[j], d[k]), fp_mul(f[((size_t)1 << log_t) + j], dr[k]));
}
__global__ __launch_bounds__(256) void k_step_coeffs(const fp *__restrict__ fac, const fp *__restrict__ d, fp *__restrict__ coeffs, unsigned log_n,
                                                     unsigned log_t) {
    const size_t k = blockIdx.x * (size_t)256 + threadIdx.x;
    coeffs[((size_t)blockIdx.y << log_n) + k] = fp_mul(fac[((size_t)blockIdx.y << log_t) + (k & (((size_t)1 << log_t) - 1))], d[k]);
}
}
hipError_t ntt_step_build_tables(uint64_t *d_d, unsigned log_block, unsigned split, const uint64_t *d_winv, const NttArgs &a, hipStream_t stream) {
    if (!ntt_step_shape(a.log_n, log_block) || a.inverse || a.width != 1 || a.in != d_d || split >= (1u << log_block)) return hipErrorInvalidValue;
    const size_t n = (size_t)1 << a.log_n;
    if (split == 0) hipLaunchKernelGGL(k_step_d, dim3((unsigned)(n / 256)), dim3(256), 0, stream, d_d, d_winv, n, a.log_n - log_block);
    else hipLaunchKernelGGL(k_step_dr, dim3((unsigned)(n / 256)), dim3(256), 0, stream, d_d, d_winv, n, split, host::from_u64(split));
    const StepPass columns_only{nullptr, nullptr, 0};
    hipError_t e = hipErrorInvalidValue;
    three_step_size(a.log_n, [&](auto split) { e = launch_three_step<decltype(split), false>(a, stream, &columns_only); });
    return e;
}
hipError_t ntt_step_coefficients(const uint64_t *d_evals, uint64_t *d_fac, uint64_t *d_coeffs, const uint64_t *d_d, unsigned ncols, unsigned log_n,
                                 unsigned log_block, const uint64_t *d_winv, uint64_t n_inv, hipStream_t stream) {
    if (!ntt_step_shape(log_n, log_block) || ncols == 0 || ncols > 65535) return hipErrorInvalidValue;
    const unsigned log_t = log_n - log_block;
    const uint64_t t_inv = host::inv(host::from_u64((uint64_t)1 << log_t));
    hipLaunchKernelGGL(k_step_factors, dim3(ncols), dim3(NT), (size_t)3 * 8 << (log_t - 1), stream, d_evals, d_fac, log_n, log_t, d_winv, n_inv, t_inv);
    hipLaunchKernelGGL(k_step_coeffs, dim3((unsigned)(((size_t)1 << log_n) / 256), ncols), dim3(256), 0, stream, (const fp *)d_fac, d_d, d_coeffs, log_n,
                       log_t);
    return hipGetLastError();
}
hipError_t ntt_step2_coefficients(const uint64_t *d_evals, uint64_t *d_fac, uint64_t *d_coeffs, const uint64_t *d_d, const uint64_t *d_dr, unsigned ncols,
                                  unsigned log_n, unsigned log_block, unsigned split, const uint64_t *d_winv, uint64_t n_inv, hipStream_t stream) {
    if (!ntt_step_shape(log_n, log_block) || ncols == 0 || ncols > 65535 || split == 0 || split >= (1u << log_block)) return hipErrorInvalidValue;
    const unsigned log_t = log_n - log_block;
    const uint64_t t_inv = host::inv(host::from_u64((uint64_t)1 << log_t));
    hipLaunchKernelGGL(k_step2_factors, dim3(ncols), dim3(NT), (size_t)5 * 8 << (log_t - 1), stream, d_evals, d_fac, log_n, log_t, split, d_winv, n_inv, t_inv);
    hipLaunchKernelGGL(k_step2_coeffs, dim3((unsigned)(((size_t)1 << log_n) / 256), ncols), dim3(256), 0, stream, (const fp *)d_fac, d_d, d_dr, d_coeffs,
                       log_n, log_t);
    return hipGetLastError();
}
hipError_t ntt_step_rows(const NttArgs &a, const uint64_t *d_wtab, const uint64_t *d_wtab_r, const uint64_t *d_fac, unsigned log_block, hipStream_t stream) {
    if (!ntt_step_shape(a.log_n, log_block) || a.inverse || !d_wtab || !d_fac) return hipErrorInvalidValue;
    const StepPass rows{d_wtab, d_fac, a.log_n - log_block, d_wtab_r};
    hipError_t e = hipErrorInvalidValue;
    three_step_size(a.log_n, [&](auto split) { e = launch_three_step<decltype(split), false>(a, stream, &rows); });
    return e;
}

hipError_t ntt_power_table(fp *d_table, size_t n, fp base, hipStream_t stream) {
    const size_t threads = (n + CHUNK - 1) / CHUNK;
    hipLaunchKernelGGL(k_power_table, dim3((unsigned)((threads + 255) / 256)), dim3(256), 0, stream, d_table, n, base);
    return hipGetLastError();
}

hipError_t ntt_columns(const NttArgs &a, hipStream_t stream) {
    if (a.log_n < NTT_MIN_LOG_N || a.log_n > NTT_MAX_LOG_N) return hipErrorInvalidValue;
    hipError_t e = hipSuccess;
    if (three_step_size(a.log_n, [&](auto split) {
            using S = decltype(split);
            e = a.inverse ? launch_three_step<S, true>(a, stream) : launch_three_step<S, false>(a, stream);
        }))
        return e;
    return (a.log_n + 1) / 2 <= 11 ? launch<8>(a, stream) : launch<4>(a, stream);
}

}
```

certificate-stark_amd/csrc/prove.hip:

```cpp
#include <hip/hip_runtime.h>
#include <string.h>
#include <algorithm>
#include <atomic>
#include <new>
#include <chrono>
#include <thread>
#include <vector>
#include "../../include/cstark.h"
#include "ctx.h"
#include "blake3.h"
#include "channel.h"
#include "deep.h"
#include "ext.h"
#include "range_batch.h"
#include "hostblake3.h"
#include "keccak.cuh"
#include "air_tx_host.h"
#include "hostfield.h"
#include "coin.h"
#include "proof_layout.h"
#include "transcript.h"

namespace cs {

enum { PROVE_EVENTS = CSTARK_PROVE_NUM_STAGES + 1 };

struct ProveArena {
    int air = -1;
    unsigned log_n = 0, log_b = 0, log_f = 0;
    uint64_t *trace = nullptr, *coeffs = nullptr, *lde = nullptr, *combined = nullptr, *ccoef = nullptr, *clde = nullptr, *deep = nullptr;
    std::vector<void *> extra;
    std::vector<size_t> extra_bytes;
    uint8_t *tnodes = nullptr, *cnodes = nullptr;
    std::vector<uint64_t *> layer;
    std::vector<uint8_t *> lnodes;
    uint32_t *d_pos = nullptr;
    uint64_t *d_pub = nullptr;
    uint64_t *d_shifts = nullptr;
    uint8_t *d_open = nullptr;
    uint64_t *h_pub = nullptr;
    uint8_t *h_open = nullptr;
    size_t h_open_bytes = 0;
    size_t open_bytes = 0;
    hipEvent_t ev[PROVE_EVENTS] = {};
    bool timed = false;
    uint32_t channel = CSTARK_CHANNEL_HOST;
    std::vector<void *> owned;
    struct ProofRun *run = nullptr;
};
void proof_run_free(struct ProofRun *r);

void prove_arena_free(ProveArena *a) {
    if (!a) return;
    proof_run_free(a->run);
    for (void *p : a->owned) (void)hipFree(p);
    if (a->h_pub) (void)hipHostFree(a->h_pub);
    if (a->h_open) (void)hipHostFree(a->h_open);
    for (hipEvent_t e : a->ev) if (e) (void)hipEventDestroy(e);
    delete a;
}
int grind_nonce(cstark_ctx *c, ProveArena *a, const Coin &coin, unsigned bits, uint64_t *nonce_out);

namespace {

__global__ void k_gather_rows(const uint64_t *__restrict__ lde, uint32_t width, uint32_t log_n, uint32_t log_b, const uint32_t *__restrict__ pos,
                              uint64_t *__restrict__ out) {
    const uint32_t q = blockIdx.x, i = pos[q], k = i & ((1u << log_b) - 1), j = i >> log_b;
    for (uint32_t c = threadIdx.x; c < width; c += blockDim.x) out[(size_t)q * width + c] = lde[(((size_t)k * width + c) << log_n) + j];
}
__global__ void k_gather_rows_window(const uint64_t *__restrict__ lde, uint32_t width, uint32_t log_n, uint32_t log_b, uint32_t k0, uint32_t nk,
                                     const uint32_t *__restrict__ pos, uint64_t *__restrict__ out, const uint64_t *__restrict__ sub, uint32_t log_nk) {
    const uint32_t q = blockIdx.x, i = pos[q], k = i & ((1u << log_b) - 1), j = i >> log_b, stride = width + 4 * log_nk;
    const bool mine = k >= k0 && k < k0 + nk;
    for (uint32_t c = threadIdx.x; c < width; c += blockDim.x)
        out[(size_t)q * stride + c] = mine ? lde[(((size_t)(k - k0) * width + c) << log_n) + j] : 0;
    const size_t leaf = ((size_t)nk << log_n) + ((size_t)j << log_nk) + (k - k0);
    for (uint32_t t = threadIdx.x; t < 4 * log_nk; t += blockDim.x)
        out[(size_t)q * stride + width + t] = mine ? sub[4 * ((leaf >> (t >> 2)) ^ 1) + (t & 3)] : 0;
}
__global__ void k_split_shard_rows(const uint64_t *__restrict__ rows, uint32_t width, uint32_t log_nk, uint32_t log_leaves, uint64_t *__restrict__ out_rows,
                                   uint64_t *__restrict__ out_paths) {
    const uint32_t q = blockIdx.x, stride = width + 4 * log_nk;
    for (uint32_t c = threadIdx.x; c < width; c += blockDim.x) out_rows[(size_t)q * width + c] = rows[(size_t)q * stride + c];
    for (uint32_t t = threadIdx.x; t < 4 * log_nk; t += blockDim.x) out_paths[(size_t)q * log_leaves * 4 + t] = rows[(size_t)q * stride + width + t];
}
__global__ void k_interleave_leaves(const uint4 *__restrict__ in, uint4 *__restrict__ out, size_t n, uint32_t log_b) {
    const size_t t = blockIdx.x * (size_t)blockDim.x + threadIdx.x;
    if (t >= (n << (log_b + 1))) return;
    const size_t i = t >> 1, half = t & 1, k = i & ((1u << log_b) - 1), j = i >> log_b;
    out[t] = in[2 * (k * n + j) + half];
}
__global__ void k_gather_paths(const uint4 *__restrict__ nodes, uint32_t log_leaves, const uint32_t *__restrict__ pos, uint4 *__restrict__ out) {
    const uint32_t q = blockIdx.x;
    for (uint32_t t = threadIdx.x; t < 2 * log_leaves; t += blockDim.x) {
        const uint32_t lvl = t >> 1, half = t & 1;
        const size_t node = ((((size_t)1 << log_leaves) + pos[q]) >> lvl) ^ 1;
// ... 6 lines not shown
__global__ void k_gather_batch(GatherBatch b) {
    const GatherJob g = b.job[blockIdx.y];
    const uint32_t q = blockIdx.x;
    if (q >= (g.dcount ? *g.dcount : g.count)) return;
    if (g.kind == 0) {
        const uint64_t *lde = (const uint64_t *)g.src;
        uint64_t *out = (uint64_t *)g.out;
        const uint32_t width = g.a, i = g.pos[q], k = lde_coset_slot(i & ((1u << g.log_b) - 1), g.log_b, g.log_s), j = i >> g.log_b;
        for (uint32_t c = threadIdx.x; c < width; c += blockDim.x) out[(size_t)q * width + c] = lde[(((size_t)k * width + c) << g.log_n) + j];
    } else {
        const uint4 *nodes = (const uint4 *)g.src;
        uint4 *out = (uint4 *)g.out;
        const uint32_t log_leaves = g.a;
        for (uint32_t t = threadIdx.x + 2 * g.lvl0; t < 2 * log_leaves; t += blockDim.x) {
            const uint32_t lvl = t >> 1, half = t & 1;
            const size_t node = ((((size_t)1 << log_leaves) + g.pos[q]) >> lvl) ^ 1;
            out[((size_t)q * log_leaves + lvl) * 2 + half] = nodes[2 * node + half];
        }
    }
}
struct GatherList {
    GatherBatch b{};
    int n = 0;
    uint32_t max_count = 0;
    void rows(const uint64_t *lde, uint32_t width, uint32_t log_n, uint32_t log_b, const uint32_t *pos, void *out, uint32_t count, uint32_t log_s = 0,
              const uint32_t *dcount = nullptr) {
        b.job[n++] = GatherJob{lde, out, pos, 0u, width, log_n, log_b, count, log_s, dcount, 0u};
        if (count > max_count) max_count = count;
    }
    void paths(const uint8_t *nodes, uint32_t log_leaves, const uint32_t *pos, void *out, uint32_t count, const uint32_t *dcount = nullptr, uint32_t lvl0 = 0) {
        b.job[n++] = GatherJob{nodes, out, pos, 1u, log_leaves, 0u, 0u, count, 0u, dcount, lvl0};
        if (count > max_count) max_count = count;
    }
    hipError_t launch(hipStream_t st) {
        if (n == 0 || max_count == 0) return hipSuccess;
        k_gather_batch<<<dim3(max_count, (unsigned)n), 128, 0, st>>>(b);
        return hipGetLastError();
    }
};
__global__ void k_gather_pub(const uint64_t *__restrict__ trace, size_t n, uint64_t *__restrict__ out, uint32_t reg0) {
    const uint32_t t = threadIdx.x;
    if (t < 14) out[t] = trace[(size_t)(reg0 + (t % 7)) * n + (t < 7 ? 0 : n - 1)];
}

template <class T>
int dev_alloc(ProveArena *a, T **p, size_t bytes) {
    HIP_TRY(hipMalloc((void **)p, bytes));
    a->owned.push_back(*p);
    return CSTARK_OK;
}

template <class T>
int arena_extra(cstark_ctx *c, ProveArena *a, size_t slot, T **p, size_t bytes) {
    if (a->extra.size() <= slot) { a->extra.resize(slot + 1, nullptr); a->extra_bytes.resize(slot + 1, 0); }
    if (a->extra[slot] && a->extra_bytes[slot] < bytes) {
        HIP_TRY(hipStreamSynchronize(c->stream));
        void *old = a->extra[slot];
        a->extra[slot] = nullptr; a->extra_bytes[slot] = 0;
        a->owned.erase(std::find(a->owned.begin(), a->owned.end(), old));
        HIP_TRY(hipFree(old));
    }
    if (!a->extra[slot]) {
        void *q;
        HIP_TRY(hipMalloc(&q, bytes));
        a->owned.push_back(q); a->extra[slot] = q; a->extra_bytes[slot] = bytes;
    }
    *p = (T *)a->extra[slot];
    return CSTARK_OK;
}

unsigned ceil_log2(uint64_t x) { unsigned l = 0; while ((1ull << l) < x) l++; return l; }

struct AirJob {
    int air = 0;
    uint32_t width = 0, log_n = 0, log_ce = 0, n_constraints = 0, n_assertions = 0, item = 0;
    std::vector<uint64_t> pub;
    std::vector<uint8_t> pub_bytes;
    int (*build)(cstark_ctx *, ProveArena *, AirJob &) = nullptr;
    int (*combine)(cstark_ctx *, ProveArena *, AirJob &, const uint64_t *ta, const uint64_t *tb, const uint64_t *ba, const uint64_t *bb, uint64_t *out) = nullptr;
    int (*combine_sets)(cstark_ctx *, ProveArena *, AirJob &, unsigned m, const uint64_t *const *ta, const uint64_t *const *tb, const uint64_t *const *ba,
                        const uint64_t *const *bb, uint64_t *const *outs) = nullptr;
    struct ColumnBatch { uint32_t col0, ncols; hipEvent_t wait[2]; uint32_t block = 0, split = 0; };
    std::vector<ColumnBatch> batches;
    const uint64_t *pub_staging = nullptr;
    bool public_ready = false;
    bool evals_ready = false;
    uint32_t k0 = 0, nk = 8;
    bool sharded = false;
    bool dev_channel = false;
    const uint64_t *d_coefs = nullptr;
    const uint64_t *d_avalues = nullptr;
    uint32_t log_b = 3;
    uint64_t seed[7] = {};
    uint64_t number = 0;
    const uint64_t *bits = nullptr;
};

void drop_run(ProveArena *a) {
    if (a && a->run) { proof_run_free(a->run); a->run = nullptr; }
}

int get_arena(cstark_ctx *c, const AirJob &job, unsigned log_b, unsigned log_f, unsigned n_layers, size_t nq, ProveArena **out) {
    drop_run(c->arena);
    if (c->arena && c->arena->air == job.air && c->arena->log_n == job.log_n && c->arena->log_b == log_b && c->arena->log_f == log_f &&
        c->arena->layer.size() == n_layers + 1 && c->arena->open_bytes >= nq) { *out = c->arena; return CSTARK_OK; }
    if (c->arena) { HIP_TRY(hipStreamSynchronize(c->stream)); prove_arena_free(c->arena); c->arena = nullptr; }
    ProveArena *a = new (std::nothrow) ProveArena();
    if (!a) return fail(CSTARK_ERR_OOM, "host allocation failed");
    c->arena = a;
    a->air = job.air; a->log_n = job.log_n; a->log_b = log_b; a->log_f = log_f;
    const size_t n = (size_t)1 << job.log_n, b = (size_t)1 << log_b, N = n * b, W = job.width, ce = (size_t)1 << job.log_ce, f = (size_t)1 << log_f;
    RC_TRY(dev_alloc(a, &a->trace, W * n * 8));
    RC_TRY(dev_alloc(a, &a->coeffs, W * n * 8));
    RC_TRY(dev_alloc(a, &a->lde, W * N * 8));
    RC_TRY(dev_alloc(a, &a->tnodes, 2 * N * 32));
    RC_TRY(dev_alloc(a, &a->combined, N * 8));
    RC_TRY(dev_alloc(a, &a->ccoef, ce * n * 8));
    RC_TRY(dev_alloc(a, &a->clde, b * ce * n * 8));
    RC_TRY(dev_alloc(a, &a->cnodes, 2 * N * 32));
    RC_TRY(dev_alloc(a, &a->deep, N * 8));
    size_t sz = N;
    for (unsigned l = 0; l <= n_layers; l++) {
        uint64_t *e; uint8_t *t = nullptr;
        RC_TRY(dev_alloc(a, &e, sz * 8));
        if (l < n_layers) RC_TRY(dev_alloc(a, &t, 2 * (sz / f) * 32));
        a->layer.push_back(e); a->lnodes.push_back(t);
        sz /= f;
    }
    RC_TRY(dev_alloc(a, &a->d_pos, 4 * 256 * (n_layers + 2)));
    RC_TRY(dev_alloc(a, &a->d_pub, 16 * 8));
    RC_TRY(dev_alloc(a, &a->d_shifts, b * 8));
    {
        std::vector<uint64_t> sh(b);
        const uint64_t wbn = host::root_of_unity(job.log_n + log_b);
        uint64_t v = host::lde_offset();
        for (size_t k = 0; k < b; k++) { sh[k] = v; v = host::mul(v, wbn); }
        HIP_TRY(hipMemcpy(a->d_shifts, sh.data(), b * 8, hipMemcpyHostToDevice));
    }
    a->open_bytes = nq;
    const size_t log_N = job.log_n + log_b;
    const size_t per_q = W * 8 + ce * 8 + 2 * log_N * 32 + (size_t)n_layers * (f * 8 + log_N * 32);
    RC_TRY(dev_alloc(a, &a->d_open, per_q * nq + 256));
    for (hipEvent_t &e : a->ev) HIP_TRY(hipEventCreate(&e));
    *out = a;
    return CSTARK_OK;
}

int check_options(const cstark_options *opt, unsigned log_ce, unsigned *log_rem_out, unsigned *log_b_out, unsigned *log_f_out) {
    const uint32_t b = opt->blowup_factor, f = opt->fri_folding_factor;
    if (b != 2 && b != 4 && b != 8 && b != 16) return fail(CSTARK_ERR_UNSUPPORTED, "blowup_factor must be 2, 4, 8 or 16");
    if (b < (1u << log_ce)) return fail(CSTARK_ERR_INVALID_ARG, "blowup_factor below the AIR's constraint-evaluation blowup (TransactionAir / SchnorrAir 8, MerkleAir 4, RangeProofAir 2)");
    if (opt->hash_fn > 1) return fail(CSTARK_ERR_UNSUPPORTED, "hash_fn must be Blake3_256 (0) or Sha3_256 (1)");
    if (opt->field_extension > 2) return fail(CSTARK_ERR_INVALID_ARG, "field_extension must be None (0), Quadratic (1) or Cubic (2)");
    if (f != 4 && f != 8 && f != 16) return fail(CSTARK_ERR_UNSUPPORTED, "fri_folding_factor must be 4, 8 or 16");
    *log_b_out = b == 2 ? 1 : b == 4 ? 2 : b == 8 ? 3 : 4;
    *log_f_out = f == 4 ? 2 : f == 8 ? 3 : 4;
    if (opt->num_queries == 0 || opt->num_queries > 128) return fail(CSTARK_ERR_INVALID_ARG, "num_queries must be 1..128");
    if (opt->grinding_factor > 32) return fail(CSTARK_ERR_INVALID_ARG, "grinding_factor must be at most 32");
    unsigned log_rem = 0;
    while ((1u << log_rem) < opt->fri_max_remainder) log_rem++;
    if ((1u << log_rem) != opt->fri_max_remainder || log_rem < 7 || log_rem > 10) return fail(CSTARK_ERR_INVALID_ARG, "fri_max_remainder must be a power of two in 128..1024");
    *log_rem_out = log_rem;
    return CSTARK_OK;
}

using transcript::channel_seed;
using transcript::SEED_PREFIX;
std::vector<uint8_t> channel_seed(const AirJob &job, const cstark_options &opt, unsigned log_rem) {
    return channel_seed(job.width, job.log_n, opt, job.log_b, log_rem, job.pub.data(), job.pub.size(), job.pub_bytes.data(), job.pub_bytes.size());
}

struct Queries {
    uint64_t nonce = 1;
    uint32_t counts[VMAX_LAYERS] = {};
    std::vector<uint32_t> hpos;
};
int query_stage(cstark_ctx *c, ProveArena *a, Coin &coin, const ProofShape &S, Queries &Q) {
    RC_TRY(grind_nonce(c, a, coin, S.opt[2], &Q.nonce));
    Q.hpos.assign(256 * (S.n_layers + 1), 0);
    transcript::draw_queries(coin, S, Q.nonce, Q.hpos.data(), Q.hpos.data() + 256, 256, Q.counts);
    HIP_TRY(hipMemcpyAsync(a->d_pos, Q.hpos.data(), Q.hpos.size() * 4, hipMemcpyHostToDevice, c->stream));
    return CSTARK_OK;
}

struct OpenBlock { size_t trows, tpaths, crows, cpaths, lrows[VMAX_LAYERS], lpaths[VMAX_LAYERS], bytes; };
OpenBlock open_block(const ProofShape &S, const uint32_t *counts, size_t start = 0, size_t align = 1) {
    OpenBlock O;
    size_t off = start;
    auto take = [&off, align](size_t bytes) { const size_t o = off; off += (bytes + align - 1) / align * align; return o; };
    O.trows = take(trace_row_bytes(S)); O.tpaths = take(path_bytes(S)); O.crows = take(comp_row_bytes(S)); O.cpaths = take(path_bytes(S));
    for (unsigned l = 0; l < S.n_layers; l++) {
        const uint32_t np = counts ? counts[l] : S.nq;
        O.lrows[l] = take(layer_row_bytes(S, np)); O.lpaths[l] = take(layer_path_bytes(S, l, np));
    }
    O.bytes = off;
    return O;
}
int host_open_block(ProveArena *a, size_t bytes) {
    if (a->h_open_bytes < bytes) {
        if (a->h_open) { HIP_TRY(hipHostFree(a->h_open)); a->h_open = nullptr; a->h_open_bytes = 0; }
        HIP_TRY(hipHostMalloc((void **)&a->h_open, bytes, hipHostMallocDefault));
        a->h_open_bytes = bytes;
    }
    return CSTARK_OK;
}
struct OpenSrc {
    const uint64_t *clde; uint64_t *const *layer; unsigned log_s;
    const uint32_t *counts, *dcount;
    const uint64_t *shard_rows; uint32_t shard_lvl0;
};
int open_stage(cstark_ctx *c, ProveArena *a, const ProofShape &S, const OpenSrc &src, uint8_t *d_block, const OpenBlock &O) {
    hipStream_t st = c->stream;
    const uint32_t nq = S.nq, W = S.width;
    GatherList gl;
    uint32_t trace_lvl0 = 0;
    if (src.shard_rows) {
        trace_lvl0 = src.shard_lvl0;
        k_split_shard_rows<<<nq, 128, 0, st>>>(src.shard_rows, W, trace_lvl0, S.log_N, (uint64_t *)(d_block + O.trows), (uint64_t *)(d_block + O.tpaths));
        HIP_TRY(hipGetLastError());
    } else gl.rows(a->lde, W, S.log_n, S.log_b, a->d_pos, d_block + O.trows, nq, src.log_s);
    gl.paths(a->tnodes, S.log_N, a->d_pos, d_block + O.tpaths, nq, nullptr, trace_lvl0);
    gl.rows(src.clde, S.ce * S.m, S.log_n, S.log_b, a->d_pos, d_block + O.crows, nq);
    gl.paths(a->cnodes, S.log_N, a->d_pos, d_block + O.cpaths, nq);
    for (unsigned l = 0; l < S.n_layers; l++) {
        const uint32_t np = src.counts ? src.counts[l] : nq, lr = layer_log_rows(S, l), *pos = a->d_pos + 256 * (l + 1), *dc = src.dcount ? src.dcount + l : nullptr;
        gl.rows(src.layer[l], S.f * S.m, lr, 0, pos, d_block + O.lrows[l], np, 0, dc);
        gl.paths(a->lnodes[l], lr, pos, d_block + O.lpaths[l], np, dc);
    }
    HIP_TRY(gl.launch(st));
    RC_TRY(host_open_block(a, O.bytes));
    HIP_TRY(hipMemcpyAsync(a->h_open, d_block, O.bytes, hipMemcpyDeviceToHost, st));
    return CSTARK_OK;
}

int lde_trace(cstark_ctx *c, ProveArena *a, const AirJob &job, uint32_t col0, uint32_t ncols) {
    const uint32_t W = job.width, log_n = job.log_n, log_b = job.log_b;
    if (job.sharded || log_b <= job.log_ce) return lde_column_range(c, a->coeffs, a->lde, W, col0, ncols, log_n, log_b, host::lde_offset(), job.k0, job.nk);
    const size_t n = (size_t)1 << log_n, ce = (size_t)1 << job.log_ce;
    const uint64_t wbn = host::root_of_unity(log_n + log_b);
    uint64_t offset = host::lde_offset();
    for (uint32_t r = 0; r < (1u << (log_b - job.log_ce)); r++) {
        RC_TRY(lde_column_range(c, a->coeffs, a->lde + (size_t)r * ce * W * n, W, col0, ncols, log_n, job.log_ce, offset, 0, (uint32_t)ce));
        offset = host::mul(offset, wbn);
    }
    return CSTARK_OK;
}
int commit_columns(cstark_ctx *c, ProveArena *a, AirJob &job, hipStream_t st, int &evi) {
    const uint32_t W = job.width, log_n = job.log_n;
    const size_t n = (size_t)1 << log_n;
    if (job.batches.empty()) {
        RC_TRY(cstark_interpolate_columns(c, a->trace, a->coeffs, W, log_n));
        HIP_TRY(hipEventRecord(a->ev[evi++], st));
        RC_TRY(lde_trace(c, a, job, 0, W));
        HIP_TRY(hipEventRecord(a->ev[evi++], st));
        return CSTARK_OK;
    }
    for (size_t i = 0; i < job.batches.size(); i++) {
        const AirJob::ColumnBatch &cb = job.batches[i];
        for (hipEvent_t e : cb.wait)
            if (e) HIP_TRY(hipStreamWaitEvent(st, e, 0));
        const bool step = cb.block != 0 && !job.sharded && job.log_b <= job.log_ce;
        if (!step) RC_TRY(cstark_interpolate_columns(c, a->trace + (size_t)cb.col0 * n, a->coeffs + (size_t)cb.col0 * n, cb.ncols, log_n));
        if (i + 1 == job.batches.size()) HIP_TRY(hipEventRecord(a->ev[evi++], st));
        if (step) RC_TRY(step_column_range(c, a->trace, a->coeffs, a->lde, W, cb.col0, cb.ncols, log_n, cb.block, cb.split, job.log_b, host::lde_offset(), job.k0, job.nk));
        else RC_TRY(lde_trace(c, a, job, cb.col0, cb.ncols));
    }
    HIP_TRY(hipEventRecord(a->ev[evi++], st));
    return CSTARK_OK;
}

}

int grind_nonce(cstark_ctx *c, ProveArena *a, const Coin &coin, unsigned bits, uint64_t *nonce_out) {
    static const bool dev_env = [] { const char *e = getenv("CSTARK_GRIND_DEVICE"); return !e || atoi(e) != 0; }();
    if (bits == 0 || !dev_env || bits < 12) {
        *nonce_out = transcript::host_nonce(coin, bits);
        return CSTARK_OK;
    }
    unsigned long long *d_found;
    RC_TRY(arena_extra(c, a, 42, &d_found, 64));
    return grind_search(c->stream, d_found, coin.seed, coin.hash_fn, bits, (uint64_t)1 << 22, nonce_out);
}
int grind_search(hipStream_t stream, unsigned long long *d_found, const uint8_t seed[32], uint32_t hash_fn, unsigned bits, uint64_t chunk, uint64_t *nonce_out) {
    if (chunk == 0) return fail(CSTARK_ERR_INVALID_ARG, "proof of work: empty chunk");
    if (hash_fn == 1) {
        HIP_TRY(hipMemcpyAsync(d_found + 1, seed, 32, hipMemcpyHostToDevice, stream));
        HIP_TRY(hipMemsetAsync(d_found, 0xFF, 8, stream));
    }
    for (uint64_t base = 1;; base += chunk) {
        if (hash_fn == 1) HIP_TRY(cs::grind_batch_chunk_sha3((const uint64_t *)(d_found + 1), 1, base, chunk, bits, d_found, stream));
        else HIP_TRY(cs::grind_chunk(seed, base, chunk, bits, d_found, stream));
        unsigned long long found = 0;
        HIP_TRY(hipMemcpyAsync(&found, d_found, 8, hipMemcpyDeviceToHost, stream));
        HIP_TRY(cs::stream_wait(stream));
        if (found != ~0ull) { *nonce_out = found; return CSTARK_OK; }
        if (base > ((uint64_t)1 << 44)) return fail(CSTARK_ERR_HIP, "proof of work: no nonce found");
    }
}

struct ProofRun {
    cstark_options opt{};
    AirJob job;
    unsigned log_rem = 0, n_layers = 0, log_b = 3, log_f = 2, m = 1;
    ProofShape shape{};
    Coin coin;
    uint8_t trace_root[32] = {}, cons_root[32] = {}, rem_commit[32] = {};
    std::vector<uint64_t> ta[3], tb[3], ba[3], bb[3], ood_trace, ood_comp, remainder;
    std::vector<uint8_t> layer_roots;
    uint64_t *comb[3] = {}, *cco[3] = {};
    uint64_t *ccoefs = nullptr;
    uint64_t *clde = nullptr, *deep = nullptr;
    std::vector<uint64_t *> layer;
    uint8_t *d_open = nullptr;
    Queries q;
    int evi = 0, phase = 0;
    bool sharded() const { return job.sharded; }
    unsigned log_s() const { return job.sharded ? 0 : log_b - job.log_ce; }
};
void proof_run_free(ProofRun *r) { delete r; }

namespace {

int run_buffers(cstark_ctx *c, ProveArena *a, ProofRun &R) {
    const unsigned m = R.m, n_layers = R.n_layers, log_N = R.job.log_n + R.log_b;
    if (m == 1) {
        R.comb[0] = a->combined; R.cco[0] = R.ccoefs = a->ccoef; R.clde = a->clde; R.deep = a->deep; R.layer = a->layer; R.d_open = a->d_open;
        return CSTARK_OK;
    }
    const size_t b = (size_t)1 << R.log_b, N = b << R.job.log_n, W = R.job.width, CN = (size_t)1 << (R.job.log_ce + R.job.log_n), nq = R.opt.num_queries;
    const uint32_t fold = 1u << R.log_f;
    uint64_t *combined_x, *ccoef_x;
    RC_TRY(arena_extra(c, a, 16, &combined_x, 2 * CN * 8));
    RC_TRY(arena_extra(c, a, 17, &ccoef_x, 2 * CN * 8));
    RC_TRY(arena_extra(c, a, 18, &R.ccoefs, 3 * CN * 8));
    RC_TRY(arena_extra(c, a, 19, &R.clde, 3 * b * CN * 8));
    RC_TRY(arena_extra(c, a, 20, &R.deep, 3 * N * 8));
    RC_TRY(arena_extra(c, a, 21, &R.d_open, nq * (W * 8 + 192 + 2 * log_N * 32 + (size_t)n_layers * (fold * 24 + log_N * 32)) + 256));
    R.layer.resize(n_layers + 1);
    size_t sz = N;
    for (unsigned l = 0; l <= n_layers; l++) { RC_TRY(arena_extra(c, a, 22 + l, &R.layer[l], 3 * sz * 8)); sz >>= R.log_f; }
    for (unsigned q = 0; q < 3; q++) { R.comb[q] = q ? combined_x + (q - 1) * CN : a->combined; R.cco[q] = q ? ccoef_x + (q - 1) * CN : a->ccoef; }
    return CSTARK_OK;
}

int run_setup(cstark_ctx *c, const cstark_options *opt, const AirJob &job, ProofRun &R, ProveArena **a) {
    RC_TRY(check_options(opt, job.log_ce, &R.log_rem, &R.log_b, &R.log_f));
    const unsigned log_N = job.log_n + R.log_b;
// ... 221 lines not shown
    const bool dev_coin = dev_coin_env && hf == 0 && m == 1 && n_layers > 0;
    uint32_t *d_fri = nullptr, *d_roots = nullptr;
    R.layer_roots.assign(32 * (size_t)n_layers, 0);
    if (dev_coin) {
        RC_TRY(arena_extra(c, a, 41, &d_fri, (size_t)(8 + 10 * 32) * 4));
        HIP_TRY(hipMemcpyAsync(d_fri, coin.seed, 32, hipMemcpyHostToDevice, st));
        d_roots = d_fri + 8 + 2 * 32;
    }
    RC_TRY(fri_commit(c, a, R, d_fri, d_roots, R.layer[n_layers]));
    R.remainder.assign((size_t)m << (log_N - n_layers * R.log_f), 0);
    if (dev_coin) HIP_TRY(hipMemcpyAsync(R.layer_roots.data(), d_roots, 32 * (size_t)n_layers, hipMemcpyDeviceToHost, st));
    HIP_TRY(hipMemcpyAsync(R.remainder.data(), R.layer[n_layers], R.remainder.size() * 8, hipMemcpyDeviceToHost, st));
    HIP_TRY(cs::stream_wait(st));
    if (dev_coin)
        for (unsigned l = 0; l < n_layers; l++) transcript::fri_layer(coin, &R.layer_roots[32 * l], m, nullptr);
    transcript::commit_remainder(coin, R.remainder.data(), R.remainder.size(), R.rem_commit);
    STAGE();

    RC_TRY(query_stage(c, a, coin, R.shape, R.q));
    R.phase = 3;
    return CSTARK_OK;
}

int phase_open(cstark_ctx *c, ProveArena *a, ProofRun &R, const uint64_t *d_trace_rows, uint8_t *proof, size_t capacity, size_t *proof_len) {
    const ProofShape &S = R.shape;
    const OpenBlock O = open_block(S, R.q.counts);
    RC_TRY(open_stage(c, a, S, {R.clde, R.layer.data(), R.log_s(), R.q.counts, nullptr, d_trace_rows, ceil_log2(R.job.nk)}, R.d_open, O));
    STAGE();
    HIP_TRY(cs::stream_wait(c->stream));
    a->timed = true; a->channel = CSTARK_CHANNEL_HOST;

    ProofParts p{};
    p.trace_root = R.trace_root; p.cons_root = R.cons_root; p.layer_roots = R.layer_roots.data(); p.rem_commit = R.rem_commit;
    p.ood_trace = R.ood_trace.data(); p.ood_comp = R.ood_comp.data(); p.nonce = R.q.nonce; p.remainder = R.remainder.data();
    return finish_proof(S, p, a->h_open, O, R.q.counts, proof, capacity, proof_len);
}

int prove_core(cstark_ctx *c, const cstark_options *opt, AirJob &job, uint8_t *proof, size_t capacity, size_t *proof_len) {
    ProofRun R;
    ProveArena *a;
    RC_TRY(run_setup(c, opt, job, R, &a));
    RC_TRY(phase_commit(c, a, R, nullptr));
    RC_TRY(phase_evaluate(c, a, R, nullptr, a->combined));
    RC_TRY(phase_compose(c, a, R));
    return phase_open(c, a, R, nullptr, proof, capacity, proof_len);
}
int prove_core_dev(cstark_ctx *c, const cstark_options *opt, AirJob &job0, uint8_t *proof, size_t capacity, size_t *proof_len) {
    const auto hp0 = std::chrono::steady_clock::now();
    ProofRun R;
    ProveArena *a;
    job0.dev_channel = true;
    RC_TRY(run_setup(c, opt, job0, R, &a));
    AirJob &job = R.job;
    const unsigned m = R.m, log_n = job.log_n, log_b = R.log_b, log_N = log_n + log_b, n_layers = R.n_layers;
    const size_t n = (size_t)1 << log_n, W = job.width, ce = (size_t)1 << job.log_ce, nq = opt->num_queries;
    const size_t rem_len = (size_t)m << (log_N - n_layers * R.log_f), n_ood = m * (2 * W + ce);
    hipStream_t st = c->stream;
    size_t off = 0;
    auto take = [&off](size_t bytes) { const size_t o = off; off += (bytes + 255) & ~(size_t)255; return o; };
    const size_t o_troot = take(32), o_croot = take(32), o_rem = take(32), o_cnt = take(4 * 64), o_ood = take(n_ood * 8), o_lroots = take(32 * (size_t)n_layers),
                 o_remainder = take(rem_len * 8);
    const ProofShape &S = R.shape;
    const OpenBlock O = open_block(S, nullptr, off, 256);
    off = O.bytes;
    uint8_t *d_res;
    uint32_t *d_fri;
    uint64_t *d_chan;
    uint64_t *sums, *dcoef;
    RC_TRY(arena_extra(c, a, 44, &d_res, off));
    RC_TRY(arena_extra(c, a, 43, &d_chan, 12 * m * 8 + n_ood * 8));
    if (m == 1) {
        RC_TRY(arena_extra(c, a, 41, &d_fri, (size_t)(8 + 10 * 32) * 4));
        RC_TRY(arena_extra(c, a, 40, &dcoef, n * 8));
        sums = R.deep;
    } else {
        RC_TRY(arena_extra(c, a, 47, &d_fri, (size_t)(8 + 2 * 3 * 32) * 4));
        RC_TRY(arena_extra(c, a, 48, &sums, 3 * n * 8));
        RC_TRY(arena_extra(c, a, 49, &dcoef, 3 * n * 8));
    }
    uint64_t *d_pts = d_chan, *d_scal = d_chan + 4 * m, *d_deepc = d_chan + 12 * m, *d_ood = (uint64_t *)(d_res + o_ood);
    uint32_t *d_cnt = (uint32_t *)(d_res + o_cnt);
    RC_TRY(host_open_block(a, off));
    RC_TRY(desc_reserve(c, ood_frames_dev_scratch_bytes((uint32_t)W, (uint32_t)ce, log_n, m)));
    uint64_t *d_coef_block;
    const bool is_tx = job.air == CSTARK_AIR_STATE_TRANSITION;
    const size_t coef_stride = is_tx ? (size_t)CE_COEF_WORDS : 230 + 2 * (size_t)job.n_assertions;
    if (is_tx) RC_TRY(tx_coef_device_block(c, &d_coef_block));
    else RC_TRY(arena_extra(c, a, 46, &d_coef_block, m * coef_stride * 8));
    const uint64_t *pw, *pwinv;
    RC_TRY(plan_tables(c, log_n, &pw, &pwinv));

    RC_TRY(commit_trace_leaves(c, a, R));
    RC_TRY(cstark_merkle_build_fn(c, R.opt.hash_fn, a->tnodes, log_N));
    STAGE();
    {
        ChanStep s{};
        s.seed = d_fri; s.m = m;
        const std::vector<uint8_t> prefix = channel_seed(job.width, log_n, *opt, log_b, R.log_rem);
        if (job.air == CSTARK_AIR_SCHNORR) {
            uint8_t key[12] = {};
            memcpy(key, prefix.data(), 2); memcpy(key + 2, prefix.data() + 10, 7); key[11] = 1;
            if (memcmp(key, c->schnorr_seed_key, sizeof key) != 0) {
                const std::vector<uint8_t> seed = channel_seed(job, *opt, R.log_rem);
                hostb3::hash(seed.data(), seed.size(), c->schnorr_seed);
                memcpy(c->schnorr_seed_key, key, sizeof key);
            }
            HIP_TRY(hipMemcpyAsync(d_fri, c->schnorr_seed, 32, hipMemcpyHostToDevice, st));
        } else {
            s.init = 1; s.pub = a->d_pub; s.npub = job.air == CSTARK_AIR_RANGE ? 1 : 14;
        }
        memcpy(s.prefix, prefix.data(), SEED_PREFIX); s.prefix_len = SEED_PREFIX;
        s.absorb[0].kind = CHAN_DIGEST; s.absorb[0].ptr = a->tnodes + 32; s.absorb[0].copy_out = d_res + o_troot;
        s.draw = CHAN_DRAW_COEFFS; s.a = job.n_constraints; s.b = job.n_assertions; s.stride = CSTARK_TX_NUM_CONSTRAINTS;
        s.set_stride = (uint32_t)coef_stride;
        s.count = (uint32_t)transcript::coefficient_draws(job.n_constraints, job.n_assertions); s.out = d_coef_block;
        HIP_TRY(channel_step(s, st));
    }
    if (is_tx) {
        RC_TRY(tx_evaluate_constraints_sets(c, a->lde, nullptr, m, nullptr, R.comb, job.item, log_n, 3, 0, 8, true, a->d_pub));
    } else {
        job.d_avalues = job.air == CSTARK_AIR_RANGE ? a->d_pub + 1 : job.air == CSTARK_AIR_SCHNORR ? nullptr : a->d_pub;
        for (unsigned q = 0; q < m; q++) {
            job.d_coefs = d_coef_block + q * coef_stride;
            RC_TRY(job.combine(c, a, job, nullptr, nullptr, nullptr, nullptr, R.comb[q]));
        }
    }
    STAGE();
    RC_TRY(commit_composition(c, a, R));
    STAGE();
    {
        ChanStep s{};
        s.seed = d_fri; s.m = m;
        s.absorb[0].kind = CHAN_DIGEST; s.absorb[0].ptr = a->cnodes + 32; s.absorb[0].copy_out = d_res + o_croot;
        s.draw = CHAN_DRAW_POINT; s.count = 1; s.b = (uint32_t)ce; s.w = host::root_of_unity(log_n); s.out = d_pts; s.out2 = d_scal;
        HIP_TRY(channel_step(s, st));
    }
    if (m == 1) RC_TRY(ood_frames_dev(c, a->coeffs, (uint32_t)W, R.ccoefs, (uint32_t)ce, log_n, d_pts, d_ood));
    else RC_TRY(ood_frames_dev_ext(c, a->coeffs, (uint32_t)W, R.ccoefs, (uint32_t)ce, log_n, m, d_pts, d_ood));
    STAGE();
    {
        ChanStep s{};
        s.seed = d_fri; s.m = m;
        s.absorb[0].kind = CHAN_ELEMS; s.absorb[0].ptr = d_ood; s.absorb[0].count = (uint32_t)(2 * m * W);
        s.absorb[1].kind = CHAN_ELEMS; s.absorb[1].ptr = d_ood + 2 * m * W; s.absorb[1].count = (uint32_t)(m * ce);
        s.draw = CHAN_DRAW_DEEP; s.a = (uint32_t)W; s.b = (uint32_t)ce; s.per = CSTARK_CONV_DEEP_DRAWS_PER_REGISTER;
        s.count = (uint32_t)transcript::deep_draws(W, ce); s.out = d_deepc; s.out2 = d_scal;
        HIP_TRY(channel_step(s, st));
    }
    if (m == 1) {
        cs::DeepParams p{};
        p.trace_lde = a->lde; p.comp_lde = R.clde; p.w = pw; p.coef = d_deepc; p.ood = d_ood; p.shifts = a->d_shifts; p.out = sums;
        p.width = (uint32_t)W; p.nb = (uint32_t)ce; p.log_n = log_n; p.k0 = 0; p.scal = d_scal;
        HIP_TRY(cs::deep_composition(p, 1, st));
    } else {
        RC_TRY(deep_composition_ext_dev(c, a->lde, R.clde, (uint32_t)W, (uint32_t)ce, m, d_deepc, d_ood, d_scal, a->d_shifts, sums, log_n, log_b, 1));
    }
    RC_TRY(deep_extend(c, R, sums, dcoef));
    const hipEvent_t deep_done = a->ev[R.evi];
    STAGE();
    RC_TRY(fri_commit(c, a, R, d_fri, (uint32_t *)(d_res + o_lroots), (uint64_t *)(d_res + o_remainder)));
    STAGE();
    {
        ChanStep s{};
        s.seed = d_fri; s.m = m;
        s.absorb[0].kind = CHAN_ELEMS; s.absorb[0].ptr = d_res + o_remainder; s.absorb[0].count = (uint32_t)rem_len; s.absorb[0].copy_out = d_res + o_rem;
        s.absorb[1].kind = CHAN_INT; s.absorb[1].value = 1;
        s.draw = CHAN_DRAW_QUERIES; s.count = (uint32_t)nq; s.log_domain = log_N; s.log_f = R.log_f; s.n_layers = n_layers; s.slot = 256;
        s.pos = a->d_pos; s.cnt = d_cnt;
        HIP_TRY(channel_step(s, st));
    }
    RC_TRY(open_stage(c, a, S, {R.clde, R.layer.data(), R.log_s(), nullptr, d_cnt + 1, nullptr, 0}, d_res, O));
    STAGE();
    static const bool hostprof = getenv("CSTARK_HOSTPROF") != nullptr;
    const auto hp1 = std::chrono::steady_clock::now();
    HIP_TRY(cs::stream_wait_tail(st, deep_done));
    const auto hp2 = std::chrono::steady_clock::now();
    a->timed = true; a->channel = CSTARK_CHANNEL_DEVICE;
    const uint8_t *h = a->h_open;
    const uint32_t *cnt = (const uint32_t *)(h + o_cnt);
    if (cnt[0] != nq) return fail(CSTARK_ERR_HIP, "device channel: the query positions could not be drawn");
    for (unsigned l = 0; l < n_layers; l++)
        if (cnt[l + 1] == 0 || cnt[l + 1] > nq) return fail(CSTARK_ERR_HIP, "device channel: bad folded position count");
    ProofParts p{};
    p.trace_root = h + o_troot; p.cons_root = h + o_croot; p.layer_roots = h + o_lroots; p.rem_commit = h + o_rem;
    p.ood_trace = h + o_ood; p.ood_comp = h + o_ood + ood_trace_bytes(S); p.remainder = h + o_remainder;
    p.nonce = 1;
    RC_TRY(finish_proof(S, p, h, O, cnt + 1, proof, capacity, proof_len));
    if (hostprof) {
        const auto hp3 = std::chrono::steady_clock::now();
        auto us = [](auto d) { return std::chrono::duration<double, std::micro>(d).count(); };
        fprintf(stderr, "[cstark hostprof] device channel: enqueued in %.0f us, waited %.0f us, proof written in %.0f us\n", us(hp1 - hp0), us(hp2 - hp1), us(hp3 - hp2));
    }
    return CSTARK_OK;
}
#undef STAGE
bool use_dev_channel(const cstark_options *opt, const AirJob &job) {
    static const bool host_env = [] { const char *e = getenv("CSTARK_HOST_CHANNEL"); return e && atoi(e) != 0; }();
    if (host_env || job.sharded || job.n_constraints > CSTARK_TX_NUM_CONSTRAINTS) return false;
    if (opt->hash_fn != 0 || opt->field_extension > 2 || opt->grinding_factor != 0) return false;
    uint32_t lb = 0, lf = 0, lr = 0;
    while ((1u << lb) < opt->blowup_factor && lb < 8) lb++;
    while ((1u << lf) < opt->fri_folding_factor && lf < 8) lf++;
    while ((1u << lr) < opt->fri_max_remainder && lr < 12) lr++;
    return lf >= 2 && job.log_n + lb > lr;
}

bool shard_split(uint32_t nk) {
    static const bool on = [] { const char *e = getenv("CSTARK_SHARD_SPLIT"); return !e || atoi(e) != 0; }();
    return on && (nk == 2 || nk == 4);
}
uint32_t shard_rows(uint32_t nk) { return shard_split(nk) ? nk / 2 + 4 : nk; }

int gather_roots(cstark_ctx *c, ProveArena *a, AirJob &job, uint32_t reg0 = 58) {
    const size_t n = (size_t)1 << job.log_n;
    k_gather_pub<<<1, 64, 0, c->stream>>>(a->trace, n, a->d_pub, reg0);
    HIP_TRY(hipGetLastError());
    if (job.dev_channel) return CSTARK_OK;
    job.pub.assign(14, 0);
    HIP_TRY(hipMemcpyAsync(job.pub.data(), a->d_pub, 14 * 8, hipMemcpyDeviceToHost, c->stream));
    return CSTARK_OK;
}


int tx_build(cstark_ctx *c, ProveArena *a, AirJob &job) {
    static const int mode = [] { const char *e = getenv("CSTARK_TRACE_OVERLAP"); return e ? atoi(e) : 1; }();
    if (mode == 0) {
        RC_TRY(cstark_tx_build_trace(c, a->trace));
        return gather_roots(c, a, job);
    }
    RC_TRY(tx_build_trace_split(c, a->trace));
    if (mode == 2) {
        for (hipEvent_t e : {c->ev_join, c->ev_mid, c->ev_join2}) HIP_TRY(hipStreamWaitEvent(c->stream, e, 0));
        return gather_roots(c, a, job);
    }
    const size_t n = (size_t)1 << job.log_n;
    if (!a->h_pub) HIP_TRY(hipHostMalloc((void **)&a->h_pub, 14 * 8, hipHostMallocDefault));
// ... 622 lines not shown
```

Measured before the change: 42.44.

## Use step-structured factors for OOD evaluation and DEEP sums of periodic-block columns

For the state-transition AIR, trace columns whose interpolant has a block-periodic step structure keep their compact step factors instead of materializing full coefficient vectors. OOD values for those columns are computed directly from the factors. The DEEP composition contribution of those columns comes from a small step-row transform of combined factors, so the generic column loop skips the gap. This removes the per-column coefficient expansion kernel and part of the poly_eval and DEEP work over 2^20-length columns. In exchange it adds arena buffers, an environment toggle and a more complex, specialized path.

```diff
diff --git a/certificate-stark_amd/csrc/capi.hip b/certificate-stark_amd/csrc/capi.hip
--- a/certificate-stark_amd/csrc/capi.hip
+++ b/certificate-stark_amd/csrc/capi.hip
@@ -225,8 +225,8 @@
     return CSTARK_OK;
 }
 int step_impl(cstark_ctx *c, uint64_t *d_evals, uint64_t *d_coeffs, uint64_t *d_lde, uint32_t width, uint32_t col0, uint32_t ncols, uint32_t log_n,
-              uint32_t block_len, uint32_t split, uint32_t log_blowup, uint64_t domain_offset, uint32_t k0, uint32_t nk) {
-    if (!c || !d_evals || !d_coeffs || !d_lde || width == 0 || ncols == 0 || (uint64_t)col0 + ncols > width)
+              uint32_t block_len, uint32_t split, uint32_t log_blowup, uint64_t domain_offset, uint32_t k0, uint32_t nk, uint64_t *d_fac_keep = nullptr) {
+    if (!c || !d_evals || (!d_coeffs && !d_fac_keep) || !d_lde || width == 0 || ncols == 0 || (uint64_t)col0 + ncols > width)
         return fail(CSTARK_ERR_INVALID_ARG, "cstark_step_columns: bad argument");
     if (log_n < cs::NTT_MIN_LOG_N || log_n > cs::NTT_MAX_LOG_N || log_blowup > 6) return fail(CSTARK_ERR_UNSUPPORTED, "unsupported domain size");
     if (block_len == 0 || (block_len & (block_len - 1)) || block_len > (1u << log_n)) return fail(CSTARK_ERR_INVALID_ARG, "the block length must be a power of two up to the trace length");
@@ -236,6 +236,7 @@
     const size_t n = (size_t)1 << log_n;
     const unsigned log_block = (unsigned)__builtin_ctz(block_len);
     if (!cs::ntt_step_shape(log_n, log_block)) {
+        if (d_fac_keep) return fail(CSTARK_ERR_INVALID_ARG, "cstark_step_columns: the factors of a shape the step transform does not serve");
         RC_TRY(interpolate_impl(c, d_evals + (size_t)col0 * n, d_coeffs + (size_t)col0 * n, ncols, log_n));
         return lde_impl(c, d_coeffs, d_lde, width, col0, ncols, log_n, log_blowup, domain_offset, k0, nk);
     }
@@ -246,13 +247,13 @@
     const cs::StepTable *tr = nullptr;
     RC_TRY(get_step_table(c, log_n, log_blowup, domain_offset, log_block, 0, &t));
     if (split) RC_TRY(get_step_table(c, log_n, log_blowup, domain_offset, log_block, split, &tr));
-    RC_TRY(ensure_ws(c, ((size_t)ncols << (log_n - log_block)) * (split ? 16 : 8)));
-    uint64_t *fac = (uint64_t *)c->ws;
+    if (!d_fac_keep) RC_TRY(ensure_ws(c, ((size_t)ncols << (log_n - log_block)) * (split ? 16 : 8)));
+    uint64_t *fac = d_fac_keep ? d_fac_keep : (uint64_t *)c->ws;
+    uint64_t *co = d_fac_keep ? nullptr : d_coeffs + (size_t)col0 * n;
     if (split)
-        HIP_TRY(cs::ntt_step2_coefficients(d_evals + (size_t)col0 * n, fac, d_coeffs + (size_t)col0 * n, t->d, tr->d, ncols, log_n, log_block, split, p->winv,
-                                           p->n_inv, c->stream));
+        HIP_TRY(cs::ntt_step2_coefficients(d_evals + (size_t)col0 * n, fac, co, t->d, tr->d, ncols, log_n, log_block, split, p->winv, p->n_inv, c->stream));
     else
-        HIP_TRY(cs::ntt_step_coefficients(d_evals + (size_t)col0 * n, fac, d_coeffs + (size_t)col0 * n, t->d, ncols, log_n, log_block, p->winv, p->n_inv, c->stream));
+        HIP_TRY(cs::ntt_step_coefficients(d_evals + (size_t)col0 * n, fac, co, t->d, ncols, log_n, log_block, p->winv, p->n_inv, c->stream));
     return lde_timed(c, (uint64_t)ncols * nk << log_n, [&] {
         cs::NttArgs a{};
         a.out = d_lde + (size_t)col0 * n; a.width = ncols; a.batch = nk; a.log_n = log_n;
@@ -644,7 +645,7 @@
     }
     uint64_t *d_pts = (uint64_t *)c->desc_buf, *d_out = d_pts + npts, *d_scr = d_out + (size_t)npts * width;
     HIP_TRY(hipMemcpyAsync(d_pts, points, (size_t)npts * 8, hipMemcpyHostToDevice, c->stream));
-    HIP_TRY(cs::poly_eval(d_coeffs, width, log_n, d_pts, npts, d_out, d_scr, c->stream));
+    HIP_TRY(cs::poly_eval(d_coeffs, width, log_n, d_pts, npts, d_out, d_scr, c->stream, cs::PolyEvalCols{step_ood_enabled()}));
     HIP_TRY(hipMemcpyAsync(out, d_out, (size_t)npts * width * 8, hipMemcpyDeviceToHost, c->stream));
     HIP_TRY(cs::stream_wait(c->stream));
     return CSTARK_OK;
@@ -778,8 +779,8 @@
     uint64_t *d_pts = (uint64_t *)c->desc_buf, *d_out = d_pts + 4, *d_scr = d_out + n_out;
     const uint64_t pts[3] = {zpts[0], zpts[1], zb};
     HIP_TRY(hipMemcpyAsync(d_pts, pts, sizeof pts, hipMemcpyHostToDevice, c->stream));
-    HIP_TRY(cs::poly_eval(d_coeffs, width, log_n, d_pts, 2, d_out, d_scr, c->stream));
-    HIP_TRY(cs::poly_eval(d_ccoef, n_comp, log_n, d_pts + 2, 1, d_out + 2 * (size_t)width, d_scr + scr_t, c->stream));
+    HIP_TRY(cs::poly_eval(d_coeffs, width, log_n, d_pts, 2, d_out, d_scr, c->stream, cs::PolyEvalCols{step_ood_enabled()}));
+    HIP_TRY(cs::poly_eval(d_ccoef, n_comp, log_n, d_pts + 2, 1, d_out + 2 * (size_t)width, d_scr + scr_t, c->stream, cs::PolyEvalCols{step_ood_enabled()}));
     std::vector<uint64_t> host(n_out);
     HIP_TRY(hipMemcpyAsync(host.data(), d_out, n_out * 8, hipMemcpyDeviceToHost, c->stream));
     HIP_TRY(cs::stream_wait(c->stream));
@@ -800,8 +801,8 @@
         c->desc_bytes = need;
     }
     uint64_t *d_scr = (uint64_t *)c->desc_buf;
-    HIP_TRY(cs::poly_eval(d_coeffs, width, log_n, d_pts, 2, d_out, d_scr, c->stream));
-    HIP_TRY(cs::poly_eval(d_ccoef, n_comp, log_n, d_pts + 2, 1, d_out + 2 * (size_t)width, d_scr + scr_t, c->stream));
+    HIP_TRY(cs::poly_eval(d_coeffs, width, log_n, d_pts, 2, d_out, d_scr, c->stream, cs::PolyEvalCols{step_ood_enabled()}));
+    HIP_TRY(cs::poly_eval(d_ccoef, n_comp, log_n, d_pts + 2, 1, d_out + 2 * (size_t)width, d_scr + scr_t, c->stream, cs::PolyEvalCols{step_ood_enabled()}));
     return CSTARK_OK;
 }
 int desc_reserve(cstark_ctx *c, size_t bytes) {
@@ -989,8 +990,55 @@
     return lde_impl(c, d_coeffs, d_lde, width, col0, ncols, log_n, log_blowup, domain_offset, k0, nk);
 }
 int step_column_range(cstark_ctx *c, uint64_t *d_evals, uint64_t *d_coeffs, uint64_t *d_lde, uint32_t width, uint32_t col0, uint32_t ncols, uint32_t log_n,
-                      uint32_t block_len, uint32_t split, uint32_t log_blowup, uint64_t domain_offset, uint32_t k0, uint32_t nk) {
-    return step_impl(c, d_evals, d_coeffs, d_lde, width, col0, ncols, log_n, block_len, split, log_blowup, domain_offset, k0, nk);
+                      uint32_t block_len, uint32_t split, uint32_t log_blowup, uint64_t domain_offset, uint32_t k0, uint32_t nk, uint64_t *d_fac_keep) {
+    return step_impl(c, d_evals, d_coeffs, d_lde, width, col0, ncols, log_n, block_len, split, log_blowup, domain_offset, k0, nk, d_fac_keep);
+}
+bool step_ood_enabled() {
+    static const bool on = [] { const char *e = getenv("CSTARK_STEP_OOD"); return !e || atoi(e) != 0; }();
+    return on;
+}
+int step_ood_tables(cstark_ctx *c, uint32_t log_n, uint32_t log_blowup, uint64_t domain_offset, uint32_t block_len, uint32_t split, cs::StepOod *s,
+                    const uint64_t **d_wtab, const uint64_t **d_wtab_r, const uint64_t **d_aux) {
+    const unsigned log_block = (unsigned)__builtin_ctz(block_len);
+    if (!cs::ntt_step_shape(log_n, log_block) || split == 0 || split >= block_len) return fail(CSTARK_ERR_INVALID_ARG, "step_ood_tables: bad shape");
+    const NttPlan *p;
+    const cs::StepTable *t, *tr;
+    RC_TRY(get_plan(c, log_n, &p));
+    RC_TRY(get_step_table(c, log_n, log_blowup, domain_offset, log_block, 0, &t));
+    RC_TRY(get_step_table(c, log_n, log_blowup, domain_offset, log_block, split, &tr));
+    s->d = t->d; s->dr = tr->d; s->log_block = log_block;
+    *d_wtab = t->w; *d_wtab_r = tr->w; *d_aux = p->aux_w;
+    return CSTARK_OK;
+}
+size_t ood_frames_step_scratch_bytes(uint32_t width, uint32_t n_comp, uint32_t log_n, uint32_t log_block) {
+    return ood_frames_dev_scratch_bytes(width, n_comp, log_n, 1) + cs::step_ood_scratch_words(log_n, log_block) * 8;
+}
+int ood_frames_dev_step(cstark_ctx *c, const uint64_t *d_coeffs, uint32_t width, const uint64_t *d_ccoef, uint32_t n_comp, uint32_t log_n,
+                        const uint64_t *d_pts, uint64_t *d_out, const cs::StepOod &s) {
+    if (!c || !d_coeffs || !d_ccoef || !d_pts || !d_out || width == 0 || n_comp == 0 || s.col2 + s.n2 != s.col1 || s.col1 + s.n1 > width ||
+        s.n1 + s.n2 >= width)
+        return fail(CSTARK_ERR_INVALID_ARG, "ood_frames_dev_step: bad argument");
+    HIP_TRY(hipSetDevice(c->device));
+    const uint32_t gap = s.n1 + s.n2, generic = width - gap;
+    const size_t scr_t = cs::poly_eval_scratch_words(generic, log_n, 2), scr_c = cs::poly_eval_scratch_words(n_comp, log_n, 1);
+    RC_TRY(desc_reserve(c, ood_frames_step_scratch_bytes(width, n_comp, log_n, s.log_block)));
+    uint64_t *d_scr = (uint64_t *)c->desc_buf;
+    HIP_TRY(cs::step_ood_values(s, width, log_n, d_pts, d_out, d_scr + scr_t + scr_c, c->stream));
+    HIP_TRY(cs::poly_eval(d_coeffs, generic, log_n, d_pts, 2, d_out, d_scr, c->stream, cs::PolyEvalCols{true, s.col2, gap}));
+    HIP_TRY(cs::poly_eval(d_ccoef, n_comp, log_n, d_pts + 2, 1, d_out + 2 * (size_t)width, d_scr + scr_t, c->stream));
+    return CSTARK_OK;
+}
+int deep_sums_step(cstark_ctx *c, cs::DeepParams p, const cs::StepOod &s, const uint64_t *d_wtab, const uint64_t *d_wtab_r, const uint64_t *d_aux,
+                   uint64_t *d_work) {
+    const size_t n = (size_t)1 << p.log_n, T = n >> s.log_block;
+    uint64_t *mfac = d_work, *consts = d_work + 4 * T, *sums = consts + 4;
+    HIP_TRY(cs::deep_step_consts(s, p.coef, p.ood, p.width, p.nb, p.log_n, mfac, consts, c->stream));
+    cs::NttArgs a{};
+    a.out = sums; a.width = 2; a.batch = 1; a.log_n = p.log_n; a.out_batch_stride = 2 * n; a.aux = d_aux;
+    HIP_TRY(cs::ntt_step_rows(a, d_wtab, d_wtab_r, mfac, s.log_block, c->stream));
+    p.step_sums = sums; p.consts = consts; p.gap_at = s.col2; p.gap_len = s.n1 + s.n2;
+    HIP_TRY(cs::deep_composition(p, 1, c->stream));
+    return CSTARK_OK;
 }
 int tx_build_trace_split(cstark_ctx *c, uint64_t *d_trace) {
     if (!c || !d_trace) return fail(CSTARK_ERR_INVALID_ARG, "tx_build_trace_split: null argument");
diff --git a/certificate-stark_amd/csrc/ctx.h b/certificate-stark_amd/csrc/ctx.h
--- a/certificate-stark_amd/csrc/ctx.h
+++ b/certificate-stark_amd/csrc/ctx.h
@@ -11,6 +11,8 @@
 
 #include <chrono>
 namespace cs {
+struct StepOod;
+struct DeepParams;
 inline hipError_t stream_wait(hipStream_t st) {
     static const bool block = [] { const char *e = getenv("CSTARK_SYNC_BLOCK"); return e && atoi(e) != 0; }();
     static const long spin_us = [] { const char *e = getenv("CSTARK_SPIN_US"); return e ? atol(e) : 200L; }();
@@ -216,7 +218,16 @@
 int lde_column_range(cstark_ctx *c, const uint64_t *d_coeffs, uint64_t *d_lde, uint32_t width, uint32_t col0, uint32_t ncols, uint32_t log_n,
                      uint32_t log_blowup, uint64_t domain_offset, uint32_t k0, uint32_t nk);
 int step_column_range(cstark_ctx *c, uint64_t *d_evals, uint64_t *d_coeffs, uint64_t *d_lde, uint32_t width, uint32_t col0, uint32_t ncols, uint32_t log_n,
-                      uint32_t block_len, uint32_t split, uint32_t log_blowup, uint64_t domain_offset, uint32_t k0, uint32_t nk);
+                      uint32_t block_len, uint32_t split, uint32_t log_blowup, uint64_t domain_offset, uint32_t k0, uint32_t nk,
+                      uint64_t *d_fac_keep = nullptr);
+bool step_ood_enabled();
+int step_ood_tables(cstark_ctx *c, uint32_t log_n, uint32_t log_blowup, uint64_t domain_offset, uint32_t block_len, uint32_t split, cs::StepOod *s,
+                    const uint64_t **d_wtab, const uint64_t **d_wtab_r, const uint64_t **d_aux);
+size_t ood_frames_step_scratch_bytes(uint32_t width, uint32_t n_comp, uint32_t log_n, uint32_t log_block);
+int ood_frames_dev_step(cstark_ctx *c, const uint64_t *d_coeffs, uint32_t width, const uint64_t *d_ccoef, uint32_t n_comp, uint32_t log_n,
+                        const uint64_t *d_pts, uint64_t *d_out, const cs::StepOod &s);
+int deep_sums_step(cstark_ctx *c, cs::DeepParams p, const cs::StepOod &s, const uint64_t *d_wtab, const uint64_t *d_wtab_r, const uint64_t *d_aux,
+                   uint64_t *d_work);
 int evaluate_ood_frames(cstark_ctx *c, const uint64_t *d_coeffs, uint32_t width, const uint64_t *d_ccoef, uint32_t n_comp, uint32_t log_n,
                         const uint64_t zpts[2], uint64_t zb, uint64_t *out_trace, uint64_t *out_comp);
 int ood_frames_dev(cstark_ctx *c, const uint64_t *d_coeffs, uint32_t width, const uint64_t *d_ccoef, uint32_t n_comp, uint32_t log_n, const uint64_t *d_pts,
diff --git a/certificate-stark_amd/csrc/debug/debug_step_ood.hip b/certificate-stark_amd/csrc/debug/debug_step_ood.hip
--- /dev/null
+++ b/certificate-stark_amd/csrc/debug/debug_step_ood.hip
@@ -0,0 +1,53 @@
+#include <hip/hip_runtime.h>
+#include "../../../include/cstark_debug_step_ood.h"
+#include "../ctx.h"
+#include "../deep.h"
+#include "../hostfield.h"
+#include "../ntt.h"
+
+extern "C" int cstark_debug_step_ood_deep(void *ctx, uint64_t *d_evals, uint64_t *d_lde, uint32_t width, uint32_t col2, uint32_t n2, uint32_t n1,
+                                          uint32_t block_len, uint32_t split, uint32_t log_n, uint32_t log_blowup, uint64_t *d_fac, const uint64_t *d_pts,
+                                          uint64_t *d_frame, const uint64_t *d_comp_lde, uint32_t n_comp, const uint64_t *d_coef, const uint64_t *d_ood,
+                                          const uint64_t *d_scal, const uint64_t *d_shifts, uint64_t *d_work, uint64_t *d_sums) {
+    cstark_ctx *c = (cstark_ctx *)ctx;
+    if (!c || !d_evals || !d_lde || !d_fac || !d_pts || !d_frame || n1 == 0 || n2 == 0 || (uint64_t)col2 + n2 + n1 > width) return CSTARK_ERR_INVALID_ARG;
+    if (block_len < 2 || (block_len & (block_len - 1)) || split == 0 || split >= block_len || log_n > cs::NTT_MAX_LOG_N || ((uint64_t)1 << log_n) <= block_len)
+        return CSTARK_ERR_INVALID_ARG;
+    if (d_coef && (!d_comp_lde || !d_ood || !d_scal || !d_shifts || !d_work || !d_sums || n_comp == 0)) return CSTARK_ERR_INVALID_ARG;
+    if (hipSetDevice(c->device) != hipSuccess) return CSTARK_ERR_HIP;
+    const unsigned log_block = (unsigned)__builtin_ctz(block_len);
+    if (!cs::ntt_step_shape(log_n, log_block)) return CSTARK_ERR_UNSUPPORTED;
+    const size_t T = ((size_t)1 << log_n) >> log_block;
+    const uint32_t col1 = col2 + n2;
+    const uint64_t off = cs::host::lde_offset();
+    cs::StepOod s;
+    s.n1 = n1; s.col1 = col1; s.n2 = n2; s.col2 = col2;
+    s.fac1 = d_fac; s.fac2 = d_fac + (size_t)n1 * T;
+    RC_TRY(desc_reserve(c, cs::step_ood_scratch_words(log_n, log_block) * 8));
+    RC_TRY(step_column_range(c, d_evals, nullptr, d_lde, width, col1, n1, log_n, block_len, 0, log_blowup, off, 0, 1, d_fac));
+    RC_TRY(step_column_range(c, d_evals, nullptr, d_lde, width, col2, n2, log_n, block_len, split, log_blowup, off, 0, 1, d_fac + (size_t)n1 * T));
+    const uint64_t *w, *wr, *aux;
+    RC_TRY(step_ood_tables(c, log_n, log_blowup, off, block_len, split, &s, &w, &wr, &aux));
+    if (cs::step_ood_values(s, width, log_n, d_pts, d_frame, (uint64_t *)c->desc_buf, c->stream) != hipSuccess) return CSTARK_ERR_HIP;
+    if (d_coef) {
+        const uint64_t *pw, *pwinv;
+        RC_TRY(plan_tables(c, log_n, &pw, &pwinv));
+        cs::DeepParams p{};
+        p.trace_lde = d_lde; p.comp_lde = d_comp_lde; p.w = pw; p.coef = d_coef; p.ood = d_ood; p.shifts = d_shifts; p.out = d_sums;
+        p.width = width; p.nb = n_comp; p.log_n = log_n; p.k0 = 0; p.scal = d_scal;
+        RC_TRY(deep_sums_step(c, p, s, w, wr, aux, d_work));
+    }
+    return hipStreamSynchronize(c->stream) == hipSuccess ? CSTARK_OK : CSTARK_ERR_HIP;
+}
+
+extern "C" int cstark_debug_poly_eval(void *ctx, const uint64_t *d_coeffs, uint32_t width, uint32_t log_n, const uint64_t *d_pts, uint32_t npts,
+                                      uint32_t tables, uint32_t gap_at, uint32_t gap_len, uint64_t *d_out) {
+    cstark_ctx *c = (cstark_ctx *)ctx;
+    if (!c || !d_coeffs || !d_pts || !d_out || width == 0 || npts == 0 || npts > 16 || log_n > 30 || (gap_len && (!tables || gap_at > width)))
+        return CSTARK_ERR_INVALID_ARG;
+    if (hipSetDevice(c->device) != hipSuccess) return CSTARK_ERR_HIP;
+    RC_TRY(desc_reserve(c, cs::poly_eval_scratch_words(width, log_n, npts) * 8));
+    if (cs::poly_eval(d_coeffs, width, log_n, d_pts, npts, d_out, (uint64_t *)c->desc_buf, c->stream, cs::PolyEvalCols{tables != 0, gap_at, gap_len}) != hipSuccess)
+        return CSTARK_ERR_HIP;
+    return hipStreamSynchronize(c->stream) == hipSuccess ? CSTARK_OK : CSTARK_ERR_HIP;
+}
diff --git a/certificate-stark_amd/csrc/deep.h b/certificate-stark_amd/csrc/deep.h
--- a/certificate-stark_amd/csrc/deep.h
+++ b/certificate-stark_amd/csrc/deep.h
@@ -14,11 +14,24 @@
     uint64_t z, zw, zb, deg_a, deg_b;
     uint32_t width, nb, log_n, k0;
     const uint64_t *scal;
+    const uint64_t *step_sums = nullptr, *consts = nullptr;
+    uint32_t gap_at = 0, gap_len = 0;
 };
 
+struct PolyEvalCols { bool tables = true; unsigned gap_at = 0, gap_len = 0; };
 size_t poly_eval_scratch_words(unsigned width, unsigned log_n, unsigned npts);
 hipError_t poly_eval(const uint64_t *d_coeffs, unsigned width, unsigned log_n, const uint64_t *d_points, unsigned npts, uint64_t *d_out,
-                     uint64_t *d_scratch, hipStream_t stream);
+                     uint64_t *d_scratch, hipStream_t stream, const PolyEvalCols &cols = PolyEvalCols());
+struct StepOod {
+    const uint64_t *fac1 = nullptr, *fac2 = nullptr, *d = nullptr, *dr = nullptr;
+    unsigned n1 = 0, col1 = 0, n2 = 0, col2 = 0, log_block = 0;
+};
+constexpr unsigned STEP_OOD_LOG_CHUNKS = 6;
+size_t step_ood_scratch_words(unsigned log_n, unsigned log_block);
+hipError_t step_ood_values(const StepOod &s, unsigned width, unsigned log_n, const uint64_t *d_points, uint64_t *d_out, uint64_t *d_scratch,
+                           hipStream_t stream);
+hipError_t deep_step_consts(const StepOod &s, const uint64_t *d_coef, const uint64_t *d_ood, unsigned width, unsigned nb, unsigned log_n, uint64_t *d_mfac,
+                            uint64_t *d_consts, hipStream_t stream);
 hipError_t deep_composition(const DeepParams &p, unsigned nk, hipStream_t stream);
 hipError_t fri_fold4(const uint64_t *d_evals, uint64_t *d_out, unsigned log_n, const uint64_t *d_winv, uint64_t offset_inv, uint64_t alpha,
                      uint64_t inv4, hipStream_t stream, const uint64_t *d_alpha = nullptr);
diff --git a/certificate-stark_amd/csrc/deep.hip b/certificate-stark_amd/csrc/deep.hip
--- a/certificate-stark_amd/csrc/deep.hip
+++ b/certificate-stark_amd/csrc/deep.hip
@@ -35,12 +35,237 @@
     }
     if (t < NP) partial[((size_t)t * width + col) * segs + seg] = part[t][0];
 }
-__global__ void k_poly_eval_sum(const fp *__restrict__ partial, fp *__restrict__ out, unsigned total, unsigned segs) {
+constexpr unsigned PE_TAB = 257;
+__global__ __launch_bounds__(256) void k_poly_eval_powers(const fp *__restrict__ points, fp *__restrict__ tab, unsigned segs, unsigned seg_len) {
+    const unsigned t = threadIdx.x;
+    const fp z = points[blockIdx.x];
+    fp *o = tab + (size_t)blockIdx.x * (PE_TAB + segs);
+    o[t] = fp_pow(z, t);
+    if (t == 0) o[256] = fp_pow(z, 256);
+    for (unsigned s = t; s < segs; s += 256) o[PE_TAB + s] = fp_pow(z, (uint64_t)s * seg_len);
+}
+template <int NP>
+__global__ __launch_bounds__(256) void k_poly_eval_partial_tab(const fp *__restrict__ coeffs, size_t n, const fp *__restrict__ tab, fp *__restrict__ partial,
+                                                               unsigned width, unsigned seg_len, unsigned gap_at, unsigned gap_len) {
+    __shared__ fp part[NP][256];
+    const unsigned segs = gridDim.x, seg = blockIdx.x, y = blockIdx.y, t = threadIdx.x;
+    const unsigned col = y + (y >= gap_at ? gap_len : 0);
+    const fp *c = coeffs + (size_t)col * n + (size_t)seg * seg_len;
+    fp z256[NP], acc[NP];
+#pragma unroll
+    for (int p = 0; p < NP; p++) { z256[p] = tab[(size_t)p * (PE_TAB + segs) + 256]; acc[p] = 0; }
+    unsigned k = (seg_len + 255) / 256;
+    for (; k >= 8; k -= 8) {
+        fp v[8];
+#pragma unroll
+        for (int i = 0; i < 8; i++) v[i] = c[(size_t)(k - 1 - i) * 256 + t];
+#pragma unroll
+        for (int i = 0; i < 8; i++) {
+#pragma unroll
+            for (int p = 0; p < NP; p++) acc[p] = fp_add(fp_mul(acc[p], z256[p]), v[i]);
+        }
+    }
+    while (k-- > 0) {
+        const fp v = k * 256 + t < seg_len ? c[(size_t)k * 256 + t] : 0;
+#pragma unroll
+        for (int p = 0; p < NP; p++) acc[p] = fp_add(fp_mul(acc[p], z256[p]), v);
+    }
+#pragma unroll
+    for (int p = 0; p < NP; p++) {
+        const fp *tp = tab + (size_t)p * (PE_TAB + segs);
+        part[p][t] = fp_mul(acc[p], fp_mul(tp[PE_TAB + seg], tp[t]));
+    }
+    __syncthreads();
+    for (int s = 128; s > 0; s >>= 1) {
+        if ((int)t < s) {
+#pragma unroll
+            for (int p = 0; p < NP; p++) part[p][t] = fp_add(part[p][t], part[p][t + s]);
+        }
+        __syncthreads();
+    }
+    if (t < NP) partial[((size_t)t * width + y) * segs + seg] = part[t][0];
+}
+__global__ void k_poly_eval_sum(const fp *__restrict__ partial, fp *__restrict__ out, unsigned total, unsigned segs, unsigned width, unsigned stride,
+                                unsigned gap_at, unsigned gap_len) {
     const unsigned i = blockIdx.x * blockDim.x + threadIdx.x;
     if (i >= total) return;
+    const fp *src = partial + (size_t)i * segs;
     fp a = 0;
-    for (unsigned s = 0; s < segs; s++) a = fp_add(a, partial[(size_t)i * segs + s]);
-    out[i] = a;
+    unsigned s = 0;
+    for (; s + 8 <= segs; s += 8) {
+        fp v[8];
+#pragma unroll
+        for (int q = 0; q < 8; q++) v[q] = src[s + q];
+#pragma unroll
+        for (int q = 0; q < 8; q++) a = fp_add(a, v[q]);
+    }
+    for (; s < segs; s++) a = fp_add(a, src[s]);
+    const unsigned p = i / width, y = i % width;
+    out[(size_t)p * stride + y + (y >= gap_at ? gap_len : 0)] = a;
+}
+
+__global__ __launch_bounds__(256) void k_step_ood_e(const fp *__restrict__ d, const fp *__restrict__ dr, const fp *__restrict__ points, fp *__restrict__ part,
+                                                    unsigned log_n, unsigned log_t, unsigned log_ch) {
+    const size_t g = blockIdx.x * (size_t)256 + threadIdx.x;
+    if (g >= ((size_t)1 << (log_t + log_ch))) return;
+    const unsigned j = (unsigned)(g & (((size_t)1 << log_t) - 1)), ch = (unsigned)(g >> log_t);
+    const unsigned per = 1u << (log_n - log_t - log_ch), i0 = ch * per;
+    fp zt[2], acc[2][2] = {{0, 0}, {0, 0}};
+#pragma unroll
+    for (int p = 0; p < 2; p++) {
+        zt[p] = points[p];
+        for (unsigned s = 0; s < log_t; s++) zt[p] = fp_sqr(zt[p]);
+    }
+    unsigned i = per;
+    for (; i >= 8; i -= 8) {
+        fp vd[8], vr[8];
+#pragma unroll
+        for (int q = 0; q < 8; q++) {
+            const size_t k = j + ((size_t)(i0 + i - 1 - q) << log_t);
+            vd[q] = d[k]; vr[q] = dr[k];
+        }
+#pragma unroll
+        for (int q = 0; q < 8; q++) {
+#pragma unroll
+            for (int p = 0; p < 2; p++) {
+                acc[p][0] = fp_add(fp_mul(acc[p][0], zt[p]), vd[q]);
+                acc[p][1] = fp_add(fp_mul(acc[p][1], zt[p]), vr[q]);
+            }
+        }
+    }
+    while (i-- > 0) {
+        const size_t k = j + ((size_t)(i0 + i) << log_t);
+        const fp vd = d[k], vr = dr[k];
+#pragma unroll
+        for (int p = 0; p < 2; p++) {
+            acc[p][0] = fp_add(fp_mul(acc[p][0], zt[p]), vd);
+            acc[p][1] = fp_add(fp_mul(acc[p][1], zt[p]), vr);
+        }
+    }
+#pragma unroll
+    for (int p = 0; p < 2; p++) {
+        const fp s = fp_pow(points[p], j + ((uint64_t)i0 << log_t));
+        fp *o = part + ((((size_t)ch * 2 + p) * 2) << log_t) + j;
+        o[0] = fp_mul(acc[p][0], s);
+        o[(size_t)1 << log_t] = fp_mul(acc[p][1], s);
+    }
+}
+__global__ __launch_bounds__(256) void k_step_ood_esum(const fp *__restrict__ part, fp *__restrict__ e, unsigned log_t, unsigned log_ch) {
+    const size_t i = blockIdx.x * (size_t)256 + threadIdx.x, words = (size_t)4 << log_t;
+    if (i >= words) return;
+    fp v[1 << STEP_OOD_LOG_CHUNKS], a = 0;
+#pragma unroll
+    for (unsigned ch = 0; ch < (1u << STEP_OOD_LOG_CHUNKS); ch++) v[ch] = ch < (1u << log_ch) ? part[ch * words + i] : 0;
+#pragma unroll
+    for (unsigned ch = 0; ch < (1u << STEP_OOD_LOG_CHUNKS); ch++) a = fp_add(a, v[ch]);
+    e[i] = a;
+}
+__global__ __launch_bounds__(256) void k_step_ood_dot(const fp *__restrict__ fac1, const fp *__restrict__ fac2, const fp *__restrict__ e, fp *__restrict__ out,
+                                                      unsigned log_t, unsigned n1, unsigned col1, unsigned col2, unsigned width) {
+    __shared__ fp part[2][256];
+    const unsigned T = 1u << log_t, t = threadIdx.x, b = blockIdx.x;
+    const bool two = b >= n1;
+    const fp *a1 = two ? fac2 + ((size_t)(b - n1) << (log_t + 1)) : fac1 + ((size_t)b << log_t);
+    Acc128 s[2] = {acc_zero(), acc_zero()};
+    for (unsigned j = t; j < T; j += 256) {
+        const fp f1 = a1[j], f2 = two ? a1[T + j] : 0;
+#pragma unroll
+        for (int p = 0; p < 2; p++) {
+            acc_mad(s[p], f1, e[(size_t)p * 2 * T + j]);
+            if (two) acc_mad(s[p], f2, e[((size_t)p * 2 + 1) * T + j]);
+            acc_fold(s[p]);
+        }
+    }
+    part[0][t] = acc_reduce(s[0]); part[1][t] = acc_reduce(s[1]);
+    __syncthreads();
+    for (int h = 128; h > 0; h >>= 1) {
+        if ((int)t < h) { part[0][t] = fp_add(part[0][t], part[0][t + h]); part[1][t] = fp_add(part[1][t], part[1][t + h]); }
+        __syncthreads();
+    }
+    if (t < 2) out[(size_t)t * width + (two ? col2 + (b - n1) : col1 + b)] = part[t][0];
+}
+
+__global__ __launch_bounds__(256) void k_deep_consts(const fp *__restrict__ coef, const fp *__restrict__ ood, const fp *__restrict__ fac1,
+                                                     const fp *__restrict__ fac2, fp *__restrict__ mfac, fp *__restrict__ consts, unsigned width,
+                                                     unsigned nb, unsigned log_t, unsigned n1, unsigned col1, unsigned n2, unsigned col2) {
+    const unsigned t = threadIdx.x, T = 1u << log_t;
+    if (blockIdx.x + 1 == gridDim.x) {
+        __shared__ fp part[3][256];
+        Acc128 s[3] = {acc_zero(), acc_zero(), acc_zero()};
+        for (unsigned c = t; c < width; c += 256) {
+            acc_mad(s[0], coef[c], ood[c]); acc_mad(s[1], coef[width + c], ood[width + c]);
+            acc_fold(s[0]); acc_fold(s[1]);
+        }
+        for (unsigned i = t; i < nb; i += 256) { acc_mad(s[2], coef[2 * width + i], ood[2 * width + i]); acc_fold(s[2]); }
+#pragma unroll
+        for (int q = 0; q < 3; q++) part[q][t] = acc_reduce(s[q]);
+        __syncthreads();
+        for (int h = 128; h > 0; h >>= 1) {
+            if ((int)t < h) {
+#pragma unroll
+                for (int q = 0; q < 3; q++) part[q][t] = fp_add(part[q][t], part[q][t + h]);
+            }
+            __syncthreads();
+        }
+        if (t < 3) consts[t] = part[t][0];
+        return;
+    }
+    const unsigned g = blockIdx.x * 256 + t;
+    if (g >= 2 * T) return;
+    const unsigned j = g & (T - 1), second = g >> log_t;
+    Acc128 sa = acc_zero(), sb = acc_zero();
+    const unsigned m1 = second ? 0 : n1, m = m1 + n2;
+    for (unsigned i0 = 0; i0 < m; i0 += 8) {
+        fp f[8], ca[8], cb[8];
+#pragma unroll
+        for (unsigned q = 0; q < 8; q++) {
+            const unsigned i = i0 + q;
+            const bool in = i < m, one = i < m1;
+            const unsigned col = one ? col1 + i : col2 + (i - m1);
+            f[q] = !in ? 0 : one ? fac1[((size_t)i << log_t) + j] : fac2[((size_t)(2 * (i - m1) + second) << log_t) + j];
+            ca[q] = in ? coef[col] : 0; cb[q] = in ? coef[width + col] : 0;
+        }
+#pragma unroll
+        for (unsigned q = 0; q < 8; q++) {
+            acc_mad(sa, ca[q], f[q]); acc_mad(sb, cb[q], f[q]);
+            if ((q & 3) == 3) { acc_fold(sa); acc_fold(sb); }
+        }
+    }
+    mfac[((size_t)second << log_t) + j] = acc_reduce(sa);
+    mfac[((size_t)(2 + second) << log_t) + j] = acc_reduce(sb);
+}
+__global__ __launch_bounds__(256) void k_deep_merged(DeepParams p) {
+    const size_t n = (size_t)1 << p.log_n;
+    const size_t j = blockIdx.x * (size_t)256 + threadIdx.x;
+    if (j >= n) return;
+    const fp x = fp_mul(p.shifts[0], p.w[j]);
+    const fp d1 = fp_sub(x, p.scal[0]), d2 = fp_sub(x, p.scal[1]), d3 = fp_sub(x, p.scal[2]);
+    const fp inv = fp_inv(fp_mul(fp_mul(d1, d2), d3));
+    const fp i1 = fp_mul(inv, fp_mul(d2, d3)), i2 = fp_mul(inv, fp_mul(d1, d3)), i3 = fp_mul(inv, fp_mul(d1, d2));
+    Acc128 s1 = acc_zero(), s2 = acc_zero(), s3 = acc_zero();
+    const fp *t = p.trace_lde + j;
+    unsigned c = 0, end = p.gap_at;
+    for (int range = 0; range < 2; range++) {
+        for (unsigned q = 0; c < end; c++, q++) {
+            const fp v = t[(size_t)c * n];
+            acc_mad(s1, p.coef[c], v);
+            acc_mad(s2, p.coef[p.width + c], v);
+            if ((q & 3) == 3) { acc_fold(s1); acc_fold(s2); }
+        }
+        acc_fold(s1); acc_fold(s2);
+        c = p.gap_at + p.gap_len; end = p.width;
+    }
+    const fp *h = p.comp_lde + j;
+    for (unsigned i = 0; i < p.nb; i++) {
+        acc_mad(s3, p.coef[2 * p.width + i], h[(size_t)i * n]);
+        if ((i & 3) == 3) acc_fold(s3);
+    }
+    acc_fold(s3);
+    const fp a1 = fp_sub(fp_add(acc_reduce(s1), p.step_sums[j]), p.consts[0]);
+    const fp a2 = fp_sub(fp_add(acc_reduce(s2), p.step_sums[n + j]), p.consts[1]);
+    const fp a3 = fp_sub(acc_reduce(s3), p.consts[2]);
+    const fp acc = fp_add(fp_add(fp_mul(a1, i1), fp_mul(a2, i2)), fp_mul(a3, i3));
+    p.out[j] = fp_mul(acc, fp_add(p.scal[3], fp_mul(p.scal[4], x)));
 }
 
 __global__ __launch_bounds__(256) void k_deep(DeepParams p) {
@@ -145,24 +370,64 @@
 
 size_t poly_eval_scratch_words(unsigned width, unsigned log_n, unsigned npts) {
     const size_t n = (size_t)1 << log_n, seg = n < (size_t)PE_SEG ? n : (size_t)PE_SEG;
-    return (size_t)npts * width * (n / seg);
+    return (size_t)npts * width * (n / seg) + (size_t)npts * (PE_TAB + n / seg);
 }
 hipError_t poly_eval(const uint64_t *d_coeffs, unsigned width, unsigned log_n, const uint64_t *d_points, unsigned npts, uint64_t *d_out,
-                     uint64_t *d_scratch, hipStream_t stream) {
+                     uint64_t *d_scratch, hipStream_t stream, const PolyEvalCols &cols) {
     const size_t n = (size_t)1 << log_n;
     const unsigned seg_len = (unsigned)(n < (size_t)PE_SEG ? n : (size_t)PE_SEG), segs = (unsigned)(n / seg_len);
+    if (cols.gap_len && (!cols.tables || cols.gap_at > width)) return hipErrorInvalidValue;
+    const unsigned stride = cols.gap_len ? width + cols.gap_len : width, gap_at = cols.gap_len ? cols.gap_at : ~0u;
+    fp *tab = d_scratch + (size_t)npts * width * segs;
+    if (cols.tables) hipLaunchKernelGGL(k_poly_eval_powers, dim3(npts), dim3(256), 0, stream, d_points, tab, segs, seg_len);
     for (unsigned p0 = 0; p0 < npts; p0 += PE_MAXPTS) {
         const unsigned np = npts - p0 >= 2 ? 2 : 1;
         fp *part = d_scratch + (size_t)p0 * width * segs;
-        if (np == 2) hipLaunchKernelGGL(k_poly_eval_partial<2>, dim3(segs, width), dim3(256), 0, stream, d_coeffs, n, d_points + p0, part, width, seg_len);
-        else hipLaunchKernelGGL(k_poly_eval_partial<1>, dim3(segs, width), dim3(256), 0, stream, d_coeffs, n, d_points + p0, part, width, seg_len);
+        const fp *tp = tab + (size_t)p0 * (PE_TAB + segs);
+        if (cols.tables) {
+            if (np == 2) hipLaunchKernelGGL(k_poly_eval_partial_tab<2>, dim3(segs, width), dim3(256), 0, stream, d_coeffs, n, tp, part, width, seg_len, gap_at, cols.gap_len);
+            else hipLaunchKernelGGL(k_poly_eval_partial_tab<1>, dim3(segs, width), dim3(256), 0, stream, d_coeffs, n, tp, part, width, seg_len, gap_at, cols.gap_len);
+        } else {
+            if (np == 2) hipLaunchKernelGGL(k_poly_eval_partial<2>, dim3(segs, width), dim3(256), 0, stream, d_coeffs, n, d_points + p0, part, width, seg_len);
+            else hipLaunchKernelGGL(k_poly_eval_partial<1>, dim3(segs, width), dim3(256), 0, stream, d_coeffs, n, d_points + p0, part, width, seg_len);
+        }
     }
     const unsigned total = npts * width;
-    hipLaunchKernelGGL(k_poly_eval_sum, dim3((total + 255) / 256), dim3(256), 0, stream, d_scratch, d_out, total, segs);
+    hipLaunchKernelGGL(k_poly_eval_sum, dim3((total + 255) / 256), dim3(256), 0, stream, d_scratch, d_out, total, segs, width, stride, gap_at, cols.gap_len);
+    return hipGetLastError();
+}
+size_t step_ood_scratch_words(unsigned log_n, unsigned log_block) {
+    const unsigned log_ch = log_block < STEP_OOD_LOG_CHUNKS ? log_block : STEP_OOD_LOG_CHUNKS;
+    return ((size_t)4 << (log_n - log_block)) * (((size_t)1 << log_ch) + 1);
+}
+hipError_t step_ood_values(const StepOod &s, unsigned width, unsigned log_n, const uint64_t *d_points, uint64_t *d_out, uint64_t *d_scratch,
+                           hipStream_t stream) {
+    if (!s.fac1 || !s.fac2 || !s.d || !s.dr || s.n1 == 0 || s.n2 == 0 || s.log_block == 0 || s.log_block >= log_n || s.col1 + s.n1 > width ||
+        s.col2 + s.n2 > width)
+        return hipErrorInvalidValue;
+    const unsigned log_t = log_n - s.log_block, log_ch = s.log_block < STEP_OOD_LOG_CHUNKS ? s.log_block : STEP_OOD_LOG_CHUNKS;
+    const size_t lanes = (size_t)1 << (log_t + log_ch), words = (size_t)4 << log_t;
+    fp *part = d_scratch, *e = d_scratch + (words << log_ch);
+    hipLaunchKernelGGL(k_step_ood_e, dim3((unsigned)((lanes + 255) / 256)), dim3(256), 0, stream, s.d, s.dr, d_points, part, log_n, log_t, log_ch);
+    hipLaunchKernelGGL(k_step_ood_esum, dim3((unsigned)((words + 255) / 256)), dim3(256), 0, stream, (const fp *)part, e, log_t, log_ch);
+    hipLaunchKernelGGL(k_step_ood_dot, dim3(s.n1 + s.n2), dim3(256), 0, stream, s.fac1, s.fac2, (const fp *)e, d_out, log_t, s.n1, s.col1, s.col2, width);
+    return hipGetLastError();
+}
+hipError_t deep_step_consts(const StepOod &s, const uint64_t *d_coef, const uint64_t *d_ood, unsigned width, unsigned nb, unsigned log_n, uint64_t *d_mfac,
+                            uint64_t *d_consts, hipStream_t stream) {
+    if (!s.fac1 || !s.fac2 || s.log_block == 0 || s.log_block >= log_n || s.col1 + s.n1 > width || s.col2 + s.n2 > width) return hipErrorInvalidValue;
+    const unsigned log_t = log_n - s.log_block;
+    hipLaunchKernelGGL(k_deep_consts, dim3((unsigned)((((size_t)2 << log_t) + 255) / 256) + 1), dim3(256), 0, stream, d_coef, d_ood, s.fac1, s.fac2, d_mfac,
+                       d_consts, width, nb, log_t, s.n1, s.col1, s.n2, s.col2);
     return hipGetLastError();
 }
 hipError_t deep_composition(const DeepParams &p, unsigned nk, hipStream_t stream) {
     const size_t n = (size_t)1 << p.log_n;
+    if (p.step_sums) {
+        if (nk != 1 || p.k0 != 0 || !p.scal || !p.consts || p.gap_at + p.gap_len > p.width) return hipErrorInvalidValue;
+        hipLaunchKernelGGL(k_deep_merged, dim3((unsigned)((n + 255) / 256)), dim3(256), 0, stream, p);
+        return hipGetLastError();
+    }
     hipLaunchKernelGGL(k_deep, dim3((unsigned)((n + 255) / 256), nk), dim3(256), 0, stream, p);
     return hipGetLastError();
 }
diff --git a/certificate-stark_amd/csrc/ntt.hip b/certificate-stark_amd/csrc/ntt.hip
--- a/certificate-stark_amd/csrc/ntt.hip
+++ b/certificate-stark_amd/csrc/ntt.hip
@@ -1216,8 +1216,9 @@
     const unsigned log_t = log_n - log_block;
     const uint64_t t_inv = host::inv(host::from_u64((uint64_t)1 << log_t));
     hipLaunchKernelGGL(k_step_factors, dim3(ncols), dim3(NT), (size_t)3 * 8 << (log_t - 1), stream, d_evals, d_fac, log_n, log_t, d_winv, n_inv, t_inv);
-    hipLaunchKernelGGL(k_step_coeffs, dim3((unsigned)(((size_t)1 << log_n) / 256), ncols), dim3(256), 0, stream, (const fp *)d_fac, d_d, d_coeffs, log_n,
-                       log_t);
+    if (d_coeffs)
+        hipLaunchKernelGGL(k_step_coeffs, dim3((unsigned)(((size_t)1 << log_n) / 256), ncols), dim3(256), 0, stream, (const fp *)d_fac, d_d, d_coeffs, log_n,
+                           log_t);
     return hipGetLastError();
 }
 hipError_t ntt_step2_coefficients(const uint64_t *d_evals, uint64_t *d_fac, uint64_t *d_coeffs, const uint64_t *d_d, const uint64_t *d_dr, unsigned ncols,
@@ -1226,8 +1227,9 @@
     const unsigned log_t = log_n - log_block;
     const uint64_t t_inv = host::inv(host::from_u64((uint64_t)1 << log_t));
     hipLaunchKernelGGL(k_step2_factors, dim3(ncols), dim3(NT), (size_t)5 * 8 << (log_t - 1), stream, d_evals, d_fac, log_n, log_t, split, d_winv, n_inv, t_inv);
-    hipLaunchKernelGGL(k_step2_coeffs, dim3((unsigned)(((size_t)1 << log_n) / 256), ncols), dim3(256), 0, stream, (const fp *)d_fac, d_d, d_dr, d_coeffs,
-                       log_n, log_t);
+    if (d_coeffs)
+        hipLaunchKernelGGL(k_step2_coeffs, dim3((unsigned)(((size_t)1 << log_n) / 256), ncols), dim3(256), 0, stream, (const fp *)d_fac, d_d, d_dr, d_coeffs,
+                           log_n, log_t);
     return hipGetLastError();
 }
 hipError_t ntt_step_rows(const NttArgs &a, const uint64_t *d_wtab, const uint64_t *d_wtab_r, const uint64_t *d_fac, unsigned log_block, hipStream_t stream) {
diff --git a/certificate-stark_amd/csrc/prove.hip b/certificate-stark_amd/csrc/prove.hip
--- a/certificate-stark_amd/csrc/prove.hip
+++ b/certificate-stark_amd/csrc/prove.hip
@@ -12,6 +12,7 @@
 #include "channel.h"
 #include "deep.h"
 #include "ext.h"
+#include "ntt.h"
 #include "range_batch.h"
 #include "hostblake3.h"
 #include "keccak.cuh"
@@ -184,6 +185,7 @@
                         const uint64_t *const *bb, uint64_t *const *outs) = nullptr;
     struct ColumnBatch { uint32_t col0, ncols; hipEvent_t wait[2]; uint32_t block = 0, split = 0; };
     std::vector<ColumnBatch> batches;
+    uint64_t *step_fac = nullptr;
     const uint64_t *pub_staging = nullptr;
     bool public_ready = false;
     bool evals_ready = false;
@@ -347,9 +349,30 @@
     }
     return CSTARK_OK;
 }
+bool step_ood_plan(const AirJob &job, StepOod *s, uint32_t *block, uint32_t *split) {
+    if (!job.step_fac || job.sharded || job.log_b > job.log_ce) return false;
+    const AirJob::ColumnBatch *one = nullptr, *two = nullptr;
+    for (const AirJob::ColumnBatch &cb : job.batches) {
+        if (cb.block == 0) continue;
+        const AirJob::ColumnBatch *&slot = cb.split ? two : one;
+        if (slot) return false;
+        slot = &cb;
+    }
+    if (!one || !two || one->block != two->block || one->block < 1024 || (one->block & (one->block - 1)) || two->col0 + two->ncols != one->col0 ||
+        !ntt_step_shape(job.log_n, (unsigned)__builtin_ctz(one->block)))
+        return false;
+    const size_t T = ((size_t)1 << job.log_n) / one->block;
+    s->n1 = one->ncols; s->col1 = one->col0; s->n2 = two->ncols; s->col2 = two->col0;
+    s->fac1 = job.step_fac; s->fac2 = job.step_fac + (size_t)one->ncols * T;
+    *block = one->block; *split = two->split;
+    return true;
+}
 int commit_columns(cstark_ctx *c, ProveArena *a, AirJob &job, hipStream_t st, int &evi) {
     const uint32_t W = job.width, log_n = job.log_n;
     const size_t n = (size_t)1 << log_n;
+    StepOod so;
+    uint32_t so_block, so_split;
+    const bool keep = step_ood_plan(job, &so, &so_block, &so_split);
     if (job.batches.empty()) {
         RC_TRY(cstark_interpolate_columns(c, a->trace, a->coeffs, W, log_n));
         HIP_TRY(hipEventRecord(a->ev[evi++], st));
@@ -364,7 +387,8 @@
         const bool step = cb.block != 0 && !job.sharded && job.log_b <= job.log_ce;
         if (!step) RC_TRY(cstark_interpolate_columns(c, a->trace + (size_t)cb.col0 * n, a->coeffs + (size_t)cb.col0 * n, cb.ncols, log_n));
         if (i + 1 == job.batches.size()) HIP_TRY(hipEventRecord(a->ev[evi++], st));
-        if (step) RC_TRY(step_column_range(c, a->trace, a->coeffs, a->lde, W, cb.col0, cb.ncols, log_n, cb.block, cb.split, job.log_b, host::lde_offset(), job.k0, job.nk));
+        if (step) RC_TRY(step_column_range(c, a->trace, a->coeffs, a->lde, W, cb.col0, cb.ncols, log_n, cb.block, cb.split, job.log_b, host::lde_offset(), job.k0, job.nk,
+                                           !keep ? nullptr : (uint64_t *)(cb.split ? so.fac2 : so.fac1)));
         else RC_TRY(lde_trace(c, a, job, cb.col0, cb.ncols));
     }
     HIP_TRY(hipEventRecord(a->ev[evi++], st));
@@ -752,6 +776,12 @@
     uint32_t *d_cnt = (uint32_t *)(d_res + o_cnt);
     RC_TRY(host_open_block(a, off));
     RC_TRY(desc_reserve(c, ood_frames_dev_scratch_bytes((uint32_t)W, (uint32_t)ce, log_n, m)));
+    uint64_t *d_step_work = nullptr;
+    if (m == 1 && job.air == CSTARK_AIR_STATE_TRANSITION && log_n >= 11 && step_ood_enabled()) {
+        RC_TRY(arena_extra(c, a, 50, &job.step_fac, 2 * W * (n >> 10) * 8));
+        RC_TRY(arena_extra(c, a, 51, &d_step_work, (4 * (n >> 10) + 4 + 2 * n) * 8));
+        RC_TRY(desc_reserve(c, ood_frames_step_scratch_bytes((uint32_t)W, (uint32_t)ce, log_n, 10)));
+    }
     uint64_t *d_coef_block;
     const bool is_tx = job.air == CSTARK_AIR_STATE_TRANSITION;
     const size_t coef_stride = is_tx ? (size_t)CE_COEF_WORDS : 230 + 2 * (size_t)job.n_assertions;
@@ -763,6 +793,11 @@
     RC_TRY(commit_trace_leaves(c, a, R));
     RC_TRY(cstark_merkle_build_fn(c, R.opt.hash_fn, a->tnodes, log_N));
     STAGE();
+    StepOod so;
+    uint32_t so_block = 0, so_split = 0;
+    const uint64_t *so_w = nullptr, *so_wr = nullptr, *so_aux = nullptr;
+    const bool step_ood = step_ood_plan(job, &so, &so_block, &so_split);
+    if (step_ood) RC_TRY(step_ood_tables(c, log_n, log_b, host::lde_offset(), so_block, so_split, &so, &so_w, &so_wr, &so_aux));
     {
         ChanStep s{};
         s.seed = d_fri; s.m = m;
@@ -805,7 +840,8 @@
         s.draw = CHAN_DRAW_POINT; s.count = 1; s.b = (uint32_t)ce; s.w = host::root_of_unity(log_n); s.out = d_pts; s.out2 = d_scal;
         HIP_TRY(channel_step(s, st));
     }
-    if (m == 1) RC_TRY(ood_frames_dev(c, a->coeffs, (uint32_t)W, R.ccoefs, (uint32_t)ce, log_n, d_pts, d_ood));
+    if (step_ood) RC_TRY(ood_frames_dev_step(c, a->coeffs, (uint32_t)W, R.ccoefs, (uint32_t)ce, log_n, d_pts, d_ood, so));
+    else if (m == 1) RC_TRY(ood_frames_dev(c, a->coeffs, (uint32_t)W, R.ccoefs, (uint32_t)ce, log_n, d_pts, d_ood));
     else RC_TRY(ood_frames_dev_ext(c, a->coeffs, (uint32_t)W, R.ccoefs, (uint32_t)ce, log_n, m, d_pts, d_ood));
     STAGE();
     {
@@ -821,7 +857,8 @@
         cs::DeepParams p{};
         p.trace_lde = a->lde; p.comp_lde = R.clde; p.w = pw; p.coef = d_deepc; p.ood = d_ood; p.shifts = a->d_shifts; p.out = sums;
         p.width = (uint32_t)W; p.nb = (uint32_t)ce; p.log_n = log_n; p.k0 = 0; p.scal = d_scal;
-        HIP_TRY(cs::deep_composition(p, 1, st));
+        if (step_ood) RC_TRY(deep_sums_step(c, p, so, so_w, so_wr, so_aux, d_step_work));
+        else HIP_TRY(cs::deep_composition(p, 1, st));
     } else {
         RC_TRY(deep_composition_ext_dev(c, a->lde, R.clde, (uint32_t)W, (uint32_t)ce, m, d_deepc, d_ood, d_scal, a->d_shifts, sums, log_n, log_b, 1));
     }
diff --git a/include/cstark_debug_step_ood.h b/include/cstark_debug_step_ood.h
--- /dev/null
+++ b/include/cstark_debug_step_ood.h
@@ -0,0 +1,17 @@
+#ifndef CSTARK_DEBUG_STEP_OOD_H
+#define CSTARK_DEBUG_STEP_OOD_H
+#include <stddef.h>
+#include <stdint.h>
+#ifdef __cplusplus
+extern "C" {
+#endif
+int cstark_debug_step_ood_deep(void *ctx, uint64_t *d_evals, uint64_t *d_lde, uint32_t width, uint32_t col2, uint32_t n2, uint32_t n1, uint32_t block_len,
+                               uint32_t split, uint32_t log_n, uint32_t log_blowup, uint64_t *d_fac, const uint64_t *d_pts, uint64_t *d_frame,
+                               const uint64_t *d_comp_lde, uint32_t n_comp, const uint64_t *d_coef, const uint64_t *d_ood, const uint64_t *d_scal,
+                               const uint64_t *d_shifts, uint64_t *d_work, uint64_t *d_sums);
+int cstark_debug_poly_eval(void *ctx, const uint64_t *d_coeffs, uint32_t width, uint32_t log_n, const uint64_t *d_pts, uint32_t npts, uint32_t tables,
+                           uint32_t gap_at, uint32_t gap_len, uint64_t *d_out);
+#ifdef __cplusplus
+}
+#endif
+#endif
```

Result: no change. 42.79 (median of 6 runs) (+0.8%).
